# nadult/Snail

Measured on AMD Instinct MI355X. Metric: Mrays/sec (primary), higher is better.
Workload: dtype f32; 1 GPU; BASELINE config 1: atrium (263124 tris, sponza.obj stand-in) 1920x1080 primary rays, hit records (t,u,v,triId); reflections=False, arith=host_sse, arith_tables=host CPU, packets=16x16 px = 1 wavefront, bvh_nodes=161677, bvh_depth=21, frames_in_flight=16, frames_per_launch=4, launches_in_flight=4, settle_frames=348, order_refresh=16, ranks=1, packet_order=heaviest first (node visits of an earlier frame), parallelism=single-gpu

## Files before the change

include/snail_hip_debug.h:

```cpp
#ifndef SNAIL_HIP_DEBUG_H
#define SNAIL_HIP_DEBUG_H
#include "snail_hip.h"
#ifdef __cplusplus
extern "C" {
#endif

int snail_debug_delay_dev(float microseconds, void *stream);

int snail_debug_clock_dev(float microseconds, uint64_t *d_out2, void *stream);

int snail_debug_recip_check(uint64_t out2[2]);

int snail_debug_hostsse_device_check(int fn, int threads, uint64_t *badChunks, uint32_t *firstBadChunk);

int snail_debug_dispatch_rate(int blocks, int threads, int reps, float *ms_per_launch);

int snail_debug_anyorder(SnailScene *, const float cam[13], int resx, int resy, int frames, int flags, float *ms_total);

int snail_debug_occupancy(int out[4]);

int snail_debug_rel_flag_count(SnailScene *, const float org[3], int *count);

#ifdef __cplusplus
}
#endif
#endif
```

snail_amd/_lib.py:

```python
from __future__ import annotations

import ctypes as C
import os

HERE = os.path.dirname(os.path.abspath(__file__))
LIB_PATH = os.environ.get("SNAIL_LIB_PATH") or os.path.join(HERE, "libsnailhip.so")


class SnailError(RuntimeError):
    pass


_lib = None

_VP, _I, _F13 = C.c_void_p, C.c_int, C.c_void_p
SIGNATURES = {
    "snail_last_error": (C.c_char_p, []),
    "snail_device_count": (_I, []),
    "snail_tris_from_verts": (_I, [_VP, _I, _VP]),
    "snail_bvh_build": (_I, [_VP, _I, _VP, _VP, _VP, _VP]),
    "snail_scene_create": (_VP, [_VP, _I, _VP, _I, _I, _I]),
    "snail_scene_destroy": (None, [_VP]),
    "snail_scene_info": (_I, [_VP, _VP, _VP, _VP, _VP]),
    "snail_scene_flags": (_I, [_VP, _VP, _VP]),
    "snail_scene_set_arith": (_I, [_VP, _I]),
    "snail_scene_arith": (_I, [_VP, _VP]),
    "snail_host_sse_tables": (_I, [_VP]),
    "snail_arith_set_tables": (_I, [_VP]),
    "snail_arith_prepare_device": (_I, []),
    "snail_host_sse_check": (_I, [_I, C.c_uint64, C.c_uint64, _I, _VP, _VP]),
    "snail_scene_create_lbvh": (_VP, [_VP, _I, _I, _I, _VP, _VP]),
    "snail_scene_download": (_I, [_VP, _VP, _VP]),
    "snail_trace_primary": (_I, [_VP, _F13, _I, _I, _I, _I, _I, _I, _VP, _VP, _VP, _VP, _VP]),
    "snail_trace_frame_packets": (_I, [_VP, _F13, _I, _I, _VP, _VP, _VP, _VP, _VP]),
    "snail_trace_primary_dev": (_I, [_VP, _F13, _I, _I, _I, _I, _I, _I, _VP, _VP, _VP, _VP, _VP, _VP]),
    "snail_trace_packets_dev": (_I, [_VP, _F13, _I, _I, _VP, _I, _VP, _VP, _VP, _VP, _VP, _VP]),
    "snail_trace_packets_shaded_dev": (_I, [_VP, _F13, _I, _I, _VP, _I, _VP, _VP, _VP]),
    "snail_trace_primary_batch_dev": (_I, [_VP, _I, _VP, _I, _I, _VP, _VP, _VP, _VP, _VP, _VP, _VP, _VP]),
    "snail_trace_packets_shaded_batch_dev": (_I, [_VP, _I, _VP, _I, _I, _VP, _I, _VP, _VP, _VP]),
    "snail_trace_primary_batch_reorder_dev": (_I, [_VP, _I, _VP, _I, _I, _VP, _VP, _VP, _VP, _VP, _VP, _VP, _VP, _I, _VP]),
    "snail_render_whitted_reorder_dev": (_I, [_VP, _F13, _I, _I, _VP, _I, _VP, _VP, _I, _VP, _I, _VP, _VP, _VP, _VP, _I, _VP]),
    "snail_primary_slots": (_I, [_I, _I]),
    "snail_trace_primary_ordered_dev": (_I, [_VP, _F13, _I, _I, _I, _I, _I, _I, _VP, _VP, _VP, _VP, _VP, _VP, _VP, _VP]),
    "snail_trace_packets_ordered_dev": (_I, [_VP, _F13, _I, _I, _VP, _I, _VP, _VP, _VP, _VP, _VP, _VP, _VP, _VP]),
    "snail_order_from_cost_dev": (_I, [_VP, _I, _VP, _VP]),
    "snail_order_from_cost_hint_dev": (_I, [_VP, _I, _VP, _I, _VP]),
    "snail_packets_to_frame_dev": (_I, [_VP, _I, _I, _I, _VP, _VP, _VP, _VP, _VP, _VP, _VP, _VP, _VP]),
    "snail_trace_rays": (_I, [_VP, _I, _I, _I, _VP, _VP, _VP, _VP, _VP, _VP, _VP, _VP]),
    "snail_trace_rays_dev": (_I, [_VP, _I, _I, _I, _VP, _VP, _VP, _VP, _VP, _VP, _VP, _VP, _VP]),
    "snail_trace_shadow": (_I, [_VP, _I, _I, _VP, _VP, _VP, _VP, _VP]),
    "snail_trace_shadow_dev": (_I, [_VP, _I, _I, _VP, _VP, _VP, _VP, _VP, _VP]),
    "snail_shade_depth_dev": (_I, [_VP, _I, _VP, _VP]),
    "snail_shade_depth_arith_dev": (_I, [_VP, _I, _VP, _I, _VP]),
    "snail_packets_bgr_to_frame_dev": (_I, [_VP, _I, _I, _I, _VP, _VP, _I, _VP]),
    "snail_packets_bgr_to_frame_chunked_dev": (_I, [_VP, _I, _I, C.c_int64, _I, _I, _VP, _VP, _I, _VP]),
    "snail_packets_bgr_to_planar_dev": (_I, [_VP, _VP, _VP, _I, _VP, _VP, _VP]),
    "snail_planar_to_frame_dev": (_I, [_VP, _VP, _I, _VP, _VP, _I, _I, _I, _VP]),
    "snail_render_whitted_dev": (_I, [_VP, _F13, _I, _I, _VP, _I, _VP, _VP, _I, _VP, _I, _VP, _VP]),
    "snail_render_whitted_ordered_dev": (_I, [_VP, _F13, _I, _I, _VP, _I, _VP, _VP, _I, _VP, _I, _VP, _VP, _VP, _VP]),
    "snail_render_whitted_packets_dev": (_I, [_VP, _F13, _I, _I, _VP, _I, _VP, _I, _VP, _VP, _I, _VP, _VP, _VP]),
    "snail_trace_transparency_dev": (_I, [_VP, _F13, _I, _I, _VP, _I, _VP, _VP, _VP, _VP, _I, _VP, _VP, _VP, _VP, _VP]),
    "snail_render_tiles": (_I, [_VP, _F13, _I, _I, _VP, _VP, _I, _VP, _I, _VP, _VP, _I, _VP, _VP]),
    "snail_render_tiles_multi": (_I, [_VP, _I, _F13, _I, _I, _VP, _VP, _I, _VP, _I, _VP, _VP, _I, _VP, _VP]),
    "snail_render_image": (_I, [_VP, _F13, _I, _I, _VP, _I, _VP, _VP, _I, _VP, _I, _VP]),
    "snail_account_primary": (_I, [_VP, _F13, _I, _I, _I, _I, _I, _I, _VP]),
    "snail_account_packets": (_I, [_VP, _F13, _I, _I, _VP]),
    "snail_last_launch": (_I, [_VP, _VP, _VP]),
}

INSTANCES_SIGNATURES = {
    "snail_instances_build": (_I, [_VP, _VP, _I, _VP, _I, _VP, _VP, _VP, _VP]),
    "snail_instances_create": (_VP, [_VP, _I, _VP, _I, _VP, _VP, _I, _I]),
    "snail_instances_update": (_I, [_VP, _VP, _I, _VP, _VP, _I, _I, _VP]),
    "snail_instances_destroy": (None, [_VP]),
    "snail_instances_trace_primary_dev": (_I, [_VP, _F13, _I, _I, _I, _I, _I, _I, _VP, _VP, _VP, _VP, _VP, _VP, _VP]),
    "snail_instances_trace_packets_dev": (_I, [_VP, _F13, _I, _I, _VP, _I, _VP, _VP, _VP, _VP, _VP, _VP, _VP]),
    "snail_instances_trace_rays_dev": (_I, [_VP, _I, _I, _I, _VP, _VP, _VP, _VP, _VP, _VP, _VP, _VP, _VP, _VP]),
    "snail_instances_trace_shadow_dev": (_I, [_VP, _I, _I, _VP, _VP, _VP, _VP, _VP, _VP]),
    "snail_instances_trace_rays": (_I, [_VP, _I, _I, _I, _VP, _VP, _VP, _VP, _VP, _VP, _VP, _VP, _VP]),
    "snail_instances_trace_shadow": (_I, [_VP, _I, _I, _VP, _VP, _VP, _VP, _VP]),
    "snail_instances_trace_frame_packets": (_I, [_VP, _F13, _I, _I, _VP, _VP, _VP, _VP, _VP, _VP]),
    "snail_instances_render_depth": (_I, [_VP, _F13, _I, _I, _VP, _I, _VP]),
}

INSTANCES_SHADE_SIGNATURES = {
    "snail_instances_render_whitted_dev": (_I, [_VP, _F13, _I, _I, _VP, _I, _VP, _VP, _I, _VP, _I, _VP, _VP]),
    "snail_instances_render_whitted_packets_dev": (_I, [_VP, _F13, _I, _I, _VP, _I, _VP, _I, _VP, _VP, _I, _VP, _VP, _VP]),
    "snail_instances_render_image": (_I, [_VP, _F13, _I, _I, _VP, _I, _VP, _VP, _I, _VP, _I, _VP]),
}

INSTANCES_TILES_SIGNATURES = {
    "snail_instances_shade_packets_dev": (_I, [_VP, _F13, _I, _I, _VP, _I, _VP, _I, _VP, _VP, _I, _VP, _VP, _VP, _VP]),
    "snail_instances_render_tiles": (_I, [_VP, _F13, _I, _I, _VP, _VP, _I, _VP, _I, _VP, _VP, _I, _VP, _VP, _VP]),
    "snail_instances_render_frame": (_I, [_VP, _F13, _I, _I, _VP, _I, _VP, _VP, _I, _VP, _I, _VP]),
}

INSTANCES_BUILD_SIGNATURES = {
    "snail_instances_rebuild_dev": (_I, [_VP, _VP, _VP, _I, _VP, _VP, _VP]),
    "snail_instances_read_tree": (_I, [_VP, _VP, _I, _VP, _VP, _VP, _I, _VP]),
}

BVH_FAST_SIGNATURES = {
    "snail_bvh_build_fast": (_I, [_VP, _I, _VP, _VP, _VP, _VP]),
    "snail_scene_create_fast_dev": (_VP, [_VP, _I, _I, _VP, _VP, _VP]),
    "snail_scene_rebuild_fast_dev": (_I, [_VP, _VP, _I, _VP, _VP, _VP]),
}

HEATMAP_SIGNATURES = {
    "snail_packet_stats_dev": (_I, [_VP, _F13, _I, _I, _VP, _I, _VP, _I, _I, _VP, _VP, _VP]),
    "snail_render_heat_packets_dev": (_I, [_VP, _F13, _I, _I, _VP, _I, _VP, _I, _I, _VP, _VP, _VP, _VP]),
    "snail_render_heat_tiles": (_I, [_VP, _F13, _I, _I, _VP, _VP, _I, _VP, _I, _I, _VP, _VP]),
    "snail_render_heat_image": (_I, [_VP, _F13, _I, _I, _VP, _I, _I, _VP, _I, _VP]),
    "snail_instances_packet_stats_dev": (_I, [_VP, _F13, _I, _I, _VP, _I, _VP, _I, _I, _VP, _VP, _VP]),
    "snail_instances_heat_packets_dev": (_I, [_VP, _F13, _I, _I, _VP, _I, _VP, _I, _I, _VP, _VP, _VP, _VP, _VP]),
    "snail_instances_render_heat_tiles": (_I, [_VP, _F13, _I, _I, _VP, _VP, _I, _VP, _I, _I, _VP, _VP, _VP]),
    "snail_instances_render_heat_frame": (_I, [_VP, _F13, _I, _I, _VP, _I, _I, _VP, _I, _VP]),
}

MATERIALS_SIGNATURES = {
    "snail_shtris_pack": (_I, [_VP, _VP, _VP, _VP, _I, _VP, _VP]),
    "snail_texture_size": (C.c_int64, [_I, _I, _VP]),
    "snail_texture_build": (_I, [_VP, _I, _I, _VP, C.c_int64, _VP]),
    "snail_materials_create": (_VP, [_VP, _VP, _I, _VP, _I, _VP, _I, _VP, _I]),
    "snail_materials_destroy": (None, [_VP]),
    "snail_materials_shade_packets_dev": (_I, [_VP, _F13, _I, _I, _VP, _I, _VP, _VP, _VP, _VP, _VP, _VP]),
    "snail_render_materials_dev": (_I, [_VP, _F13, _I, _I, _VP, _I, _VP, _I, _VP, _I, _VP, _VP]),
    "snail_render_materials_packets_dev": (_I, [_VP, _F13, _I, _I, _VP, _I, _VP, _I, _VP, _I, _VP, _VP, _VP]),
    "snail_render_materials_image": (_I, [_VP, _F13, _I, _I, _VP, _I, _VP, _I, _VP, _I, _VP]),
}

MATERIALS_BOUNCE_SIGNATURES = {
    "snail_materials_mirror_packets_dev": (_I, [_VP, _F13, _I, _I, _VP, _I, _VP, _VP, _VP, _VP, _VP, _VP, _VP, _VP, _VP, _VP]),
    "snail_materials_shade_rays_dev": (_I, [_VP, _I, _VP, _VP, _VP, _VP, _VP, _VP, _VP, _VP]),
    "snail_materials_bounce_dev": (_I, [_VP, _F13, _I, _I, _VP, _I, _VP, _I, _VP, _I, _VP, _VP]),
    "snail_materials_bounce_packets_dev": (_I, [_VP, _F13, _I, _I, _VP, _I, _VP, _I, _VP, _I, _VP, _VP, _VP]),
    "snail_materials_bounce_image": (_I, [_VP, _F13, _I, _I, _VP, _I, _VP, _I, _VP, _I, _VP]),
}

MATERIALS_TILES_SIGNATURES = {
    "snail_materials_frame_packets_dev": (_I, [_VP, _F13, _I, _I, _VP, _I, _VP, _I, _VP, _I, _VP, _VP, _VP, _VP]),
    "snail_materials_render_tiles": (_I, [_VP, _F13, _I, _I, _VP, _VP, _I, _VP, _I, _VP, _I, _VP, _VP, _VP]),
    "snail_materials_render_frame": (_I, [_VP, _F13, _I, _I, _VP, _I, _VP, _I, _VP, _I, _VP]),
}

DEBUG_SIGNATURES = {
    "snail_debug_delay_dev": (_I, [C.c_float, _VP]),
    "snail_debug_clock_dev": (_I, [C.c_float, _VP, _VP]),
    "snail_debug_recip_check": (_I, [_VP]),
    "snail_debug_dispatch_rate": (_I, [_I, _I, _I, _VP]),
    "snail_debug_hostsse_device_check": (_I, [_I, _I, _VP, _VP]),
    "snail_debug_occupancy": (_I, [_VP]),
    "snail_debug_anyorder": (_I, [_VP, _F13, _I, _I, _I, _I, _VP]),
    "snail_debug_rel_flag_count": (_I, [_VP, _VP, _VP]),
}
DEBUG_LIB_PATH = os.path.join(HERE, "libsnailhip_debug.so")
_dbg = None


def debug_lib():
    global _dbg
    if _dbg is None:
        if not os.path.exists(DEBUG_LIB_PATH):
            raise SnailError("workbench library %s is missing: `make -C snail_amd/csrc debug`" % DEBUG_LIB_PATH)
        L = C.CDLL(DEBUG_LIB_PATH)
        for table in (SIGNATURES, INSTANCES_SIGNATURES, INSTANCES_SHADE_SIGNATURES, INSTANCES_TILES_SIGNATURES, INSTANCES_BUILD_SIGNATURES, BVH_FAST_SIGNATURES, HEATMAP_SIGNATURES, MATERIALS_SIGNATURES, MATERIALS_BOUNCE_SIGNATURES, MATERIALS_TILES_SIGNATURES, DEBUG_SIGNATURES):
            for name, (res, args) in table.items():
                fn = getattr(L, name)
                fn.restype = res
                fn.argtypes = args
        _dbg = L
    return _dbg


def lib():
    global _lib
    if _lib is None:
        if not os.path.exists(LIB_PATH):
            raise SnailError(
                "HIP extension %s is missing: run `python -c 'import __graft_entry__ as g; g.build()'` "
                "(or `make -C snail_amd/csrc`). There is no CPU fallback." % LIB_PATH)
        try:
            L = C.CDLL(LIB_PATH)
        except OSError as e:
            raise SnailError("cannot load %s: %s" % (LIB_PATH, e)) from e
        for table in (SIGNATURES, INSTANCES_SIGNATURES, INSTANCES_SHADE_SIGNATURES, INSTANCES_TILES_SIGNATURES, INSTANCES_BUILD_SIGNATURES, BVH_FAST_SIGNATURES, HEATMAP_SIGNATURES, MATERIALS_SIGNATURES, MATERIALS_BOUNCE_SIGNATURES, MATERIALS_TILES_SIGNATURES):
            for name, (res, args) in table.items():
                fn = getattr(L, name)
                fn.restype = res
                fn.argtypes = args
        for name, (res, args) in DEBUG_SIGNATURES.items():
            fn = getattr(L, name, None)
            if fn is not None:
                fn.restype = res
                fn.argtypes = args
        _lib = L
    return _lib


def check(rc: int, what: str) -> None:
    if rc != 0:
        msg = lib().snail_last_error()
        raise SnailError("%s failed (status %d): %s" % (what, rc, msg.decode() if msg else "?"))


def ptr(a):
    if a is None:
        return None
    if hasattr(a, "data_ptr"):
        return C.c_void_p(a.data_ptr())
    return a.ctypes.data_as(C.c_void_p)
```

snail_amd/csrc/bvh_fast.inc:

```
namespace devf {

using devb::BuildHdr;
using devb::TNode;
static_assert(SNAIL_MAX_DEPTH == devb::kMaxDepth, "BuildHdr::qCount and the small kernel's stack are sized for DBVH::maxDepth == BVH::maxDepth");

struct FastArgs : devb::SplitArgs {
	const float *verts;
	uint4 *nodes, *pf, *tris;
	unsigned trisOff;
	int needSane;
	int *cur;
	int *perm, *info;
};

__global__ void k_fast_init(FastArgs A) {
	const int i = blockIdx.x * blockDim.x + threadIdx.x;
	if(i < A.n) A.startCnt[i] = 0;
	if(i == 0) devb::hdrInit(*A.hdr);
}

__global__ void k_fast_boxes(FastArgs A) {
	const int i = blockIdx.x * blockDim.x + threadIdx.x;
	if(i >= A.n) return;
	float p[9], rec[16];
// ... 13 lines not shown
	for(int k = 0; k < 3; k++) { o[k] = lo[k]; o[3 + k] = hi[k]; }
	A.src[i] = i;
	for(int k = 0; k < 3; k++) { devb::keyMin(&A.hdr->rootMin[k], lo[k], i); devb::keyMax(&A.hdr->rootMax[k], hi[k], i); }
}

__global__ void k_fast_commit(FastArgs A) {
	const BuildHdr &H = *A.hdr;
	const int g = blockIdx.x * blockDim.x + threadIdx.x, stride = gridDim.x * blockDim.x;
	const int status = H.status != 0 ? H.status : (A.needSane && H.insane) ? 3 : 0;
	if(status != 0) {
		if(g == 0 && A.info) { A.info[0] = status; A.info[1] = 0; A.info[2] = 0; A.info[3] = A.n; }
		return;
	}
	const int nTemp = H.nTemp;
	for(int t = g; t < nTemp; t += stride) {
		const TNode nd = A.tn[t];
		const int idx = t == 0 ? 0 : 1 + 2 * (A.startCnt[nd.pfirst] + nd.pchain) + nd.side;
		const unsigned sub = nd.inner ? (unsigned)(1 + 2 * (A.startCnt[nd.first] + nd.chain)) : ((unsigned)nd.first | 0x80000000u);
		const unsigned in[8] = {__float_as_uint(nd.lo[0]), __float_as_uint(nd.lo[1]), __float_as_uint(nd.lo[2]), __float_as_uint(nd.hi[0]),
								__float_as_uint(nd.hi[1]), __float_as_uint(nd.hi[2]), sub, (unsigned)nd.aux};
		A.nodes[(size_t)idx * 2] = make_uint4(in[0], in[1], in[2], in[3]);
		A.nodes[(size_t)idx * 2 + 1] = make_uint4(in[4], in[5], in[6], in[7]);
		if(A.pf) {
			unsigned out[8];
			dev::pfEncode(in, out, A.trisOff);
			A.pf[(size_t)(idx + 1) * 2] = make_uint4(out[0], out[1], out[2], out[3]);
			A.pf[(size_t)(idx + 1) * 2 + 1] = make_uint4(out[4], out[5], out[6], out[7]);
		}
	}
	for(int i = g; i < A.n; i += stride) {
		const int s = A.src[i];
		float p[9], rec[16];
		for(int k = 0; k < 9; k++) p[k] = A.verts[(size_t)s * 9 + k];
		(void)dev::lbvh::triRecord(p, rec);
		uint4 *o = A.tris + (size_t)i * 4;
		for(int q = 0; q < 4; q++)
			o[q] = make_uint4(__float_as_uint(rec[q * 4]), __float_as_uint(rec[q * 4 + 1]), __float_as_uint(rec[q * 4 + 2]), __float_as_uint(rec[q * 4 + 3]));
		if(A.perm) A.perm[i] = s;
	}
	if(g == 0) {
		const int nNodes = 1 + 2 * H.totalInner;
		A.cur[0] = nNodes; A.cur[1] = H.depth; A.cur[2] = H.insane ? 0 : 1; A.cur[3] = 0;
		if(A.info) { A.info[0] = 0; A.info[1] = nNodes; A.info[2] = H.depth; A.info[3] = A.n; }
	}
}

}

struct SnailSceneFast {
	char *base = nullptr;
	int *dCur = nullptr;
	int cur[4] = {0, 0, 0, 0};
	bool curOnDevice = false;
	int depthLimit = SNAIL_MAX_DEPTH;
	hipEvent_t ready = nullptr;
	bool hasReady = false;
	struct Use { hipStream_t stream; hipEvent_t ev; };
	std::vector<Use> uses;
};

namespace {

void fastFree(SnailSceneFast *f) {
	if(!f) return;
	if(f->base) (void)hipFree(f->base);
	if(f->dCur) (void)hipFree(f->dCur);
	if(f->ready) (void)hipEventDestroy(f->ready);
	for(auto &u : f->uses) (void)hipEventDestroy(u.ev);
	delete f;
}

int fastSceneBegin(SnailScene *s, hipStream_t stream) {
	SnailSceneFast *f = s->fast;
	if(f->hasReady) HIP_TRY(hipStreamWaitEvent(stream, f->ready, 0));
	return 0;
}
void fastSceneEnd(SnailScene *s, hipStream_t stream) {
	SnailSceneFast *f = s->fast;
	for(auto &u : f->uses)
		if(u.stream == stream) { (void)hipEventRecord(u.ev, stream); return; }
	SnailSceneFast::Use u;
	u.stream = stream;
	if(hipEventCreateWithFlags(&u.ev, hipEventDisableTiming) != hipSuccess) return;
	(void)hipEventRecord(u.ev, stream);
	f->uses.push_back(u);
}

int fastEnqueue(SnailScene *s, const float *dVerts, int32_t *dPerm, int32_t *dInfo, int needSane, hipStream_t st) {
	SnailSceneFast *f = s->fast;
	const int n = s->nTris;
	devf::FastArgs A;
	memset((void *)&A, 0, sizeof(A));
	buildCarve(f->base, n, A);
	A.n = n; A.maxDepth = f->depthLimit;
	A.verts = dVerts;
	A.nodes = s->dNodes; A.tris = s->dTris; A.pf = s->pfOKButNesting ? (uint4 *)s->dPF : nullptr; A.trisOff = (unsigned)s->trisOff;
	A.needSane = needSane; A.cur = f->dCur; A.perm = dPerm; A.info = dInfo;
	const devb::SplitArgs &SA = A;
	typedef devb::SplitBvh P;
	const int perN = (n + 255) / 256;
	hipLaunchKernelGGL(devf::k_fast_init, dim3(perN), dim3(256), 0, st, A);
	hipLaunchKernelGGL(devf::k_fast_boxes, dim3(perN), dim3(256), 0, st, A);
	hipLaunchKernelGGL(devb::k_build_root<P>, dim3(1), dim3(64), 0, st, SA);
	if(n > devb::kSmall) {
		const int most = n / (devb::kSmall + 1) + 1;
		const int wide = 28;
		for(int level = 0; level < wide; level++) {
			const int grid = std::min(level < 11 ? (1 << level) : 2048, most);
			hipLaunchKernelGGL(devb::k_build_big<P>, dim3(grid), dim3(256), 0, st, SA, level, level + 1);
		}
		hipLaunchKernelGGL(devb::k_build_big<P>, dim3(1), dim3(256), 0, st, SA, wide, (int)devb::kLevels);
	}
	if(n >= P::minSplit) hipLaunchKernelGGL(devb::k_build_small<P>, dim3(std::min(n / 2 + 1, 8192)), dim3(64), 0, st, SA);
	hipLaunchKernelGGL(devb::k_build_scan, dim3(1), dim3(1024), 0, st, SA);
	hipLaunchKernelGGL(devf::k_fast_commit, dim3((unsigned)std::min((2 * (long long)n + 255) / 256, 4096LL)), dim3(256), 0, st, A);
	HIP_TRY(hipGetLastError());
	if(!f->ready) HIP_TRY(hipEventCreateWithFlags(&f->ready, hipEventDisableTiming));
	HIP_TRY(hipEventRecord(f->ready, st));
	f->hasReady = true;
	f->curOnDevice = true;
	return 0;
}

int fastCurrent(const SnailScene *cs, int cur[4]) {
	SnailScene *s = const_cast<SnailScene *>(cs);
	SnailSceneFast *f = s->fast;
	DeviceGuard guard(s->device);
	std::lock_guard<std::mutex> lock(s->mu);
	if(f->curOnDevice) {
		if(f->hasReady) HIP_TRY(hipEventSynchronize(f->ready));
		HIP_TRY(hipMemcpy(f->cur, f->dCur, sizeof(f->cur), hipMemcpyDeviceToHost));
		f->curOnDevice = false;
	}
	memcpy(cur, f->cur, sizeof(f->cur));
	return 0;
}

}

extern "C" {

SnailScene *snail_scene_create_fast_dev(const float *d_verts9, int nTris, int device, int32_t *d_perm, int32_t *d_info, void *stream) {
	const char *fn = "snail_scene_create_fast_dev";
	if(!d_verts9 || nTris <= 0 || nTris > (1 << 29)) { snail_set_error("%s: bad arguments", fn); return nullptr; }
	DeviceGuard guard(device);
	if(!guard.ok) { snail_set_error("%s: hipSetDevice(%d) failed", fn, device); return nullptr; }
	hipStream_t st = (hipStream_t)stream;
	SnailScene *s = new SnailScene();
	s->fast = new SnailSceneFast();
	SnailSceneFast *f = s->fast;
	const int cap = 2 * nTris - 1;
	s->device = device; s->nNodes = cap; s->nTris = nTris;
	const size_t trisOff = pfTrisOffset(cap), pfBytes = trisOff + (size_t)nTris * 64;
	const bool fits = (size_t)cap + 1 < ((size_t)1 << 20) && pfBytes < ((size_t)1 << 31);
	s->trisOff = (int)(fits ? trisOff : 0);
	s->pfOKButNesting = fits ? 1 : 0;
	hipError_t e;
	if((e = hipMalloc((void **)&s->dNodes, (size_t)cap * 32)) != hipSuccess || (e = hipMalloc((void **)&s->dPF, fits ? pfBytes : (size_t)nTris * 64)) != hipSuccess ||
	   (e = hipMalloc((void **)&f->base, buildScratchBytes(nTris))) != hipSuccess || (e = hipMalloc((void **)&f->dCur, 4 * sizeof(int))) != hipSuccess ||
	   (fits && (e = hipMemset(s->dPF, 0, ((size_t)cap + 1) * 32)) != hipSuccess) || (e = hipMemset(f->dCur, 0, 4 * sizeof(int))) != hipSuccess) {
		snail_set_error("%s: %s", fn, hipGetErrorString(e));
		snail_scene_destroy(s);
		return nullptr;
	}
	s->dTris = (uint4 *)(s->dPF + s->trisOff);
	hipLaunchKernelGGL(dev::lbvh::k_fill_empty, dim3((unsigned)((cap + 255) / 256)), dim3(256), 0, 0, (float *)s->dNodes, cap);
	int cur[4] = {0, 0, 0, 0}, status[8] = {0};
	if((e = hipDeviceSynchronize()) != hipSuccess || fastEnqueue(s, d_verts9, d_perm, d_info, 0, st) != 0 || (e = hipStreamSynchronize(st)) != hipSuccess ||
	   (e = hipMemcpy(status, f->base, sizeof(status), hipMemcpyDeviceToHost)) != hipSuccess || fastCurrent(s, cur) != 0) {
		if(e != hipSuccess) snail_set_error("%s: %s", fn, hipGetErrorString(e));
		snail_scene_destroy(s);
		return nullptr;
	}
	if(status[0] != 0) {
		if(status[0] == 1) snail_set_error("%s: a vertex is not finite", fn);
		else snail_set_error("%s: the tree is deeper than BVH::maxDepth = %d", fn, SNAIL_MAX_DEPTH);
		snail_scene_destroy(s);
		return nullptr;
	}
	s->depth = cur[1]; s->fastOK = cur[2]; s->nestedOK = 1; s->pfOK = s->pfOKButNesting;
	f->depthLimit = s->depth > 62 ? SNAIL_MAX_DEPTH : 62;
	return s;
}

int snail_scene_rebuild_fast_dev(SnailScene *s, const float *d_verts9, int nTris, int32_t *d_perm, int32_t *d_info, void *stream) {
	const char *fn = "snail_scene_rebuild_fast_dev";
	if(int rc = checkScene(s, fn)) return rc;
	if(!s->fast) { snail_set_error("%s: the handle was not made by snail_scene_create_fast_dev", fn); return 1; }
	if(!d_verts9 || nTris != s->nTris) { snail_set_error("%s: %d triangles, the handle holds %d (or null vertices)", fn, nTris, s->nTris); return 1; }
	hipStream_t st = (hipStream_t)stream;
	DeviceGuard guard(s->device);
	SNAIL_LOCK(s);
	SnailSceneFast *f = s->fast;
	for(auto &u : f->uses) HIP_TRY(hipStreamWaitEvent(st, u.ev, 0));
	if(f->hasReady) HIP_TRY(hipStreamWaitEvent(st, f->ready, 0));
	for(auto &e : s->rel) e.valid = false;
	return fastEnqueue(s, d_verts9, d_perm, d_info, s->fastOK, st);
}

}
```

snail_amd/csrc/snail_dev.inc:

```
namespace SNAIL_DEV_NS {

typedef unsigned long long u64;
typedef unsigned u32x4 __attribute__((ext_vector_type(4)));
typedef const __attribute__((address_space(4))) u32x4 *scalar_ptr;

struct Node {
	float bmin[3], bmax[3];
	unsigned sub;
	int aux;
};

__device__ __forceinline__ float asf(unsigned u) { return __uint_as_float(u); }
__device__ __forceinline__ float asf(int u) { return __int_as_float(u); }

typedef const __attribute__((address_space(4))) char *scalar_bytes;
__device__ __forceinline__ Node loadNode(const uint4 *nodes, int idx) {
	const unsigned off = (unsigned)idx << 5;
	scalar_ptr p = (scalar_ptr)((scalar_bytes)(unsigned long long)nodes + off);
	u32x4 a = p[0], b = p[1];
	Node n;
	n.bmin[0] = asf(a.x); n.bmin[1] = asf(a.y); n.bmin[2] = asf(a.z);
	n.bmax[0] = asf(a.w); n.bmax[1] = asf(b.x); n.bmax[2] = asf(b.y);
	n.sub = b.z; n.aux = (int)b.w;
	return n;
// ... 721 lines not shown
		const int farIdx = (int)n.sub + (firstNode ^ 1);
		const Node nn = loadNode(nodes, nearIdx);

		auto fastPass = [&](const Node &n) -> u64 {
			float tn[4], tf[4];
			if(M == M_COH) {
				float pn[3], pf[3];
#pragma unroll
				for(int k = 0; k < 3; k++) {
					const int lo = __float_as_int(n.bmin[k]), hi = __float_as_int(n.bmax[k]);
					const int sw = (lo ^ hi) & octMask[k];
					pn[k] = __int_as_float(lo ^ sw); pf[k] = __int_as_float(hi ^ sw);
					if(SHARED) { pn[k] = pn[k] - org[k][0]; pf[k] = pf[k] - org[k][0]; }
				}
#pragma unroll
				for(int l = 0; l < 4; l++) {
					float lo[3], hi[3];
#pragma unroll
					for(int k = 0; k < 3; k++) {
						lo[k] = Q.id[k][l] * (SHARED ? pn[k] : pn[k] - org[k][l]);
						hi[k] = Q.id[k][l] * (SHARED ? pf[k] : pf[k] - org[k][l]);
					}
					tn[l] = vmax3(lo[0], lo[1], lo[2]);
					tf[l] = vmin3(hi[0], hi[1], hi[2]);
				}
			} else {
				float pn[3], pf[3];
#pragma unroll
				for(int k = 0; k < 3; k++) { pn[k] = SHARED ? n.bmin[k] - org[k][0] : n.bmin[k]; pf[k] = SHARED ? n.bmax[k] - org[k][0] : n.bmax[k]; }
#pragma unroll
				for(int l = 0; l < 4; l++) {
					float lo[3], hi[3];
#pragma unroll
					for(int k = 0; k < 3; k++) {
						const float a = Q.id[k][l] * (SHARED ? pn[k] : pn[k] - org[k][l]);
						const float b = Q.id[k][l] * (SHARED ? pf[k] : pf[k] - org[k][l]);
						lo[k] = vmin(a, b); hi[k] = vmax(a, b);
					}
					tn[l] = vmax3(lo[0], lo[1], lo[2]);
					tf[l] = vmin3(hi[0], hi[1], hi[2]);
				}
			}
			if(DISTPOS) {
#pragma unroll
				for(int l = 0; l < 4; l++) { tn[l] = vmax(tn[l], 0.0f); tf[l] = vmin(tf[l], Q.dist[l]); }
				const float slack = vmax3(tf[0] - tn[0], tf[1] - tn[1], vmax(tf[2] - tn[2], tf[3] - tn[3]));
				return __builtin_amdgcn_ballot_w64(slack >= 0.0f);
			} else {
				float sl[4];
#pragma unroll
				for(int l = 0; l < 4; l++) sl[l] = vmin(vmin(tf[l], Q.dist[l]) - tn[l], tf[l]);
				const float slack = vmax3(sl[0], sl[1], vmax(sl[2], sl[3]));
				return __builtin_amdgcn_ballot_w64(slack >= 0.0f);
			}
				};
		u64 passMask = 0;
		if(EXACT) {
			bool anyPass = false;
			if(boxTestInterval(n, iv)) {
				float tmn[3], tmx[3];
				if(SHARED) {
#pragma unroll
					for(int k = 0; k < 3; k++) { tmn[k] = n.bmin[k] - org[k][0]; tmx[k] = n.bmax[k] - org[k][0]; }
				}
#pragma unroll
				for(int l = 0; l < 4; l++) {
					float lmin = 0.0f, lmax = 0.0f;
#pragma unroll
					for(int k = 0; k < 3; k++) {
						float l1 = Q.id[k][l] * (SHARED ? tmn[k] : n.bmin[k] - org[k][l]);
						float l2 = Q.id[k][l] * (SHARED ? tmx[k] : n.bmax[k] - org[k][l]);
						float lo = Min<M_EXACT>(l1, l2), hi = Max<M_EXACT>(l1, l2);
						if(k == 0) { lmin = lo; lmax = hi; }
						else if(SHADOW) { lmin = Max<M_EXACT>(lo, lmin); lmax = Min<M_EXACT>(hi, lmax); }
						else { lmin = Max<M_EXACT>(lmin, lo); lmax = Min<M_EXACT>(lmax, hi); }
					}
					bool pass = SHADOW ? (lmax >= 0.0f && lmin <= Min<M_EXACT>(lmax, Q.dist[l])) : !(lmax < 0.0f || lmin > Min<M_EXACT>(lmax, Q.dist[l]));
					anyPass |= pass;
				}
			}
			passMask = __builtin_amdgcn_ballot_w64(anyPass);
		} else passMask = fastPass(n);
		const u64 alive = passMask & __builtin_amdgcn_ballot_w64((unsigned)(lane - first) <= (unsigned)(last - first));
		if(alive != 0) {
			first = __builtin_ctzll(alive);
			last = 63 - __builtin_clzll(alive);
			if(!isLeaf) {
				const int fl = first | (last << 8);
				if(!DEEP || sp < 64) writeLane2(stkNode, farIdx, stkFL, fl, sp);
				else writeLane2(stkNode2, farIdx, stkFL2, fl, sp - 64);
				sp++;
				n = nn;
				continue;
			}
		const int count = n.aux, firstTri = (int)(n.sub & 0x7fffffffu);
		if(SHARED) {
			if(leafShared<MASK, SHADOW, M, BARY>(tris, count, firstTri, size, lane, first, last, org, Q, mask4, tid, bu, bv, iv, st)) return;
		} else {
			leafPerRay<MASK, M, BARY>(tris, count, firstTri, lane, first, last, org, Q, mask4, tid, bu, bv, st);
		}
		}
		if(sp == 0) break;
		sp--;
		int cur, fl;
		if(!DEEP || sp < 64) { cur = __builtin_amdgcn_readlane(stkNode, sp); fl = __builtin_amdgcn_readlane(stkFL, sp); }
		else { cur = __builtin_amdgcn_readlane(stkNode2, sp - 64); fl = __builtin_amdgcn_readlane(stkFL2, sp - 64); }
		first = fl & 0xff; last = fl >> 8;
		n = loadNode(nodes, cur);
	}
}

#define SNAIL_SLAB_COH(L, NX, FX, NY, FY, NZ, FZ)                                                                                           \
	"v_mul_f32 %[t0], %[ix" L "], %[pnx]\n v_mul_f32 %[t1], %[iy" L "], %[pny]\n v_mul_f32 %[t2], %[iz" L "], %[pnz]\n"                    \
	"v_mul_f32 %[t3], %[ix" L "], %[pfx]\n v_mul_f32 %[t4], %[iy" L "], %[pfy]\n v_mul_f32 %[t5], %[iz" L "], %[pfz]\n"                    \
	"v_max3_f32 %[t0], %[t0], %[t1], %[t2]\n v_min3_f32 %[t3], %[t3], %[t4], %[t5]\n"
#define SNAIL_SLAB_FAST(L, NX, FX, NY, FY, NZ, FZ)                                                                                          \
	"v_mul_f32 %[t0], %[ix" L "], %[pnx]\n v_mul_f32 %[t3], %[ix" L "], %[pfx]\n v_min_f32 %[u0], %[t0], %[t3]\n v_max_f32 %[t3], %[t0], %[t3]\n" \
	"v_mul_f32 %[t1], %[iy" L "], %[pny]\n v_mul_f32 %[t4], %[iy" L "], %[pfy]\n v_min_f32 %[t0], %[t1], %[t4]\n v_max_f32 %[t4], %[t1], %[t4]\n" \
	"v_mul_f32 %[t2], %[iz" L "], %[pnz]\n v_mul_f32 %[t5], %[iz" L "], %[pfz]\n v_min_f32 %[t1], %[t2], %[t5]\n v_max_f32 %[t5], %[t2], %[t5]\n" \
	"v_max3_f32 %[t0], %[u0], %[t0], %[t1]\n v_min3_f32 %[t3], %[t3], %[t4], %[t5]\n"
#define SNAIL_SLAB_COH_R(L, NX, FX, NY, FY, NZ, FZ)                                                                                         \
	"v_mul_f32 %[t0], " NX ", %[ix" L "]\n v_mul_f32 %[t1], " NY ", %[iy" L "]\n v_mul_f32 %[t2], " NZ ", %[iz" L "]\n"                    \
	"v_mul_f32 %[t3], " FX ", %[ix" L "]\n v_mul_f32 %[t4], " FY ", %[iy" L "]\n v_mul_f32 %[t5], " FZ ", %[iz" L "]\n"                    \
	"v_max3_f32 %[t0], %[t0], %[t1], %[t2]\n v_min3_f32 %[t3], %[t3], %[t4], %[t5]\n"
#define SNAIL_SLAB_FAST_R(L, NX, FX, NY, FY, NZ, FZ)                                                                                        \
	"v_mul_f32 %[t0], " NX ", %[ix" L "]\n v_mul_f32 %[t3], " FX ", %[ix" L "]\n v_min_f32 %[u0], %[t0], %[t3]\n v_max_f32 %[t3], %[t0], %[t3]\n" \
	"v_mul_f32 %[t1], " NY ", %[iy" L "]\n v_mul_f32 %[t4], " FY ", %[iy" L "]\n v_min_f32 %[t0], %[t1], %[t4]\n v_max_f32 %[t4], %[t1], %[t4]\n" \
	"v_mul_f32 %[t2], " NZ ", %[iz" L "]\n v_mul_f32 %[t5], " FZ ", %[iz" L "]\n v_min_f32 %[t1], %[t2], %[t5]\n v_max_f32 %[t5], %[t2], %[t5]\n" \
	"v_max3_f32 %[t0], %[u0], %[t0], %[t1]\n v_min3_f32 %[t3], %[t3], %[t4], %[t5]\n"
#define SNAIL_SLABO_COH(L, NX, FX, NY, FY, NZ, FZ)                                                                                          \
	"v_sub_f32 %[t0], " NX ", %[ox" L "]\n v_sub_f32 %[t1], " NY ", %[oy" L "]\n v_sub_f32 %[t2], " NZ ", %[oz" L "]\n"                    \
	"v_sub_f32 %[t3], " FX ", %[ox" L "]\n v_sub_f32 %[t4], " FY ", %[oy" L "]\n v_sub_f32 %[t5], " FZ ", %[oz" L "]\n"                    \
	"v_mul_f32 %[t0], %[ix" L "], %[t0]\n v_mul_f32 %[t1], %[iy" L "], %[t1]\n v_mul_f32 %[t2], %[iz" L "], %[t2]\n"                       \
	"v_mul_f32 %[t3], %[ix" L "], %[t3]\n v_mul_f32 %[t4], %[iy" L "], %[t4]\n v_mul_f32 %[t5], %[iz" L "], %[t5]\n"                       \
	"v_max3_f32 %[t0], %[t0], %[t1], %[t2]\n v_min3_f32 %[t3], %[t3], %[t4], %[t5]\n"
#define SNAIL_SLABO_FAST(L, NX, FX, NY, FY, NZ, FZ)                                                                                         \
	"v_sub_f32 %[t0], " NX ", %[ox" L "]\n v_sub_f32 %[t3], " FX ", %[ox" L "]\n v_mul_f32 %[t0], %[ix" L "], %[t0]\n v_mul_f32 %[t3], %[ix" L "], %[t3]\n" \
	"v_min_f32 %[u0], %[t0], %[t3]\n v_max_f32 %[t3], %[t0], %[t3]\n"                                                                      \
	"v_sub_f32 %[t1], " NY ", %[oy" L "]\n v_sub_f32 %[t4], " FY ", %[oy" L "]\n v_mul_f32 %[t1], %[iy" L "], %[t1]\n v_mul_f32 %[t4], %[iy" L "], %[t4]\n" \
	"v_min_f32 %[t0], %[t1], %[t4]\n v_max_f32 %[t4], %[t1], %[t4]\n"                                                                      \
	"v_sub_f32 %[t2], " NZ ", %[oz" L "]\n v_sub_f32 %[t5], " FZ ", %[oz" L "]\n v_mul_f32 %[t2], %[iz" L "], %[t2]\n v_mul_f32 %[t5], %[iz" L "], %[t5]\n" \
	"v_min_f32 %[t1], %[t2], %[t5]\n v_max_f32 %[t5], %[t2], %[t5]\n"                                                                      \
	"v_max3_f32 %[t0], %[u0], %[t0], %[t1]\n v_min3_f32 %[t3], %[t3], %[t4], %[t5]\n"
#define SNAIL_PRE_SHARED(NX, FX, NY, FY, NZ, FZ)                                                                                            \
	" v_sub_f32 %[pnx], " NX ", %[ox]\n v_sub_f32 %[pny], " NY ", %[oy]\n v_sub_f32 %[pnz], " NZ ", %[oz]\n"                               \
	" v_sub_f32 %[pfx], " FX ", %[ox]\n v_sub_f32 %[pfy], " FY ", %[oy]\n v_sub_f32 %[pfz], " FZ ", %[oz]\n"
#define SNAIL_PRE_NONE(NX, FX, NY, FY, NZ, FZ) ""
#define SNAIL_ORG_SHARED() [ox] "v"(org[0][0]), [oy] "v"(org[1][0]), [oz] "v"(org[2][0])
#define SNAIL_ORG_PERRAY()                                                                                                                 \
	[ox0] "v"(org[0][0]), [ox1] "v"(org[0][1]), [ox2] "v"(org[0][2]), [ox3] "v"(org[0][3]), [oy0] "v"(org[1][0]), [oy1] "v"(org[1][1]),     \
		[oy2] "v"(org[1][2]), [oy3] "v"(org[1][3]), [oz0] "v"(org[2][0]), [oz1] "v"(org[2][1]), [oz2] "v"(org[2][2]), [oz3] "v"(org[2][3])
#define SNAIL_TAIL_POS(L, S) "v_max_f32 %[t0], 0, %[t0]\n v_min_f32 %[t3], %[t3], %[d" L "]\n v_sub_f32 %[" S "], %[t3], %[t0]\n"
#define SNAIL_TAIL_ANY(L, S) "v_min_f32 %[t4], %[t3], %[d" L "]\n v_sub_f32 %[t4], %[t4], %[t0]\n v_min_f32 %[" S "], %[t4], %[t3]\n"
#define SNAIL_POP_2W                                                                                                                       \
	" v_readlane_b32 %[cur], %[stkN], %[sp]\n v_readlane_b32 %[fl], %[stkF], %[sp]\n"                                                      \
	" s_and_b32 %[first], %[fl], 0xff\n s_lshr_b32 %[last], %[fl], 8\n"
#define SNAIL_PUSH_2W                                                                                                                      \
	" s_lshl_b32 %[off], %[last], 8\n s_or_b32 %[off], %[off], %[first]\n"                                                                 \
	" s_mov_b32 m0, %[sp]\n v_writelane_b32 %[stkN], %[fl], m0\n v_writelane_b32 %[stkF], %[off], m0\n"
#define SNAIL_COUNT " s_add_u32 %[cnt], %[cnt], 1\n"
#define SNAIL_DRAIN_SMEM " s_waitcnt lgkmcnt(0)\n"
#define SNAIL_DESCEND_ASM(PRE, ORGOPS, SLAB, TAIL, CNTPOP, CNTVISIT, NX, FX, NY, FY, NZ, FZ)                                                 \
	asm volatile(SNAIL_DRAIN_SMEM                                                                                                          \
				 "L_pop_%=:\n"                                                                                                             \
				 " s_cmp_eq_u32 %[sp], 0\n s_cbranch_scc1 L_done_%=\n"                                                                     \
				 " s_sub_u32 %[sp], %[sp], 1\n" CNTPOP                                                                                     \
				 SNAIL_POP_2W                                                                                                              \
				 " s_lshl_b32 %[off], %[cur], 5\n s_load_dwordx8 s[84:91], %[base], %[off]\n"                                              \
				 " s_sub_u32 %[width], %[last], %[first]\n"                                                                                \
				 " s_bfm_b64 exec, %[width], %[first]\n s_bitset1_b64 exec, %[last]\n"                                                     \
				 " s_waitcnt lgkmcnt(0)\n"                                                                                                 \
				 "L_visit_%=:\n" CNTVISIT                                                                                                  \
				 PRE(NX, FX, NY, FY, NZ, FZ)                                                                                               \
				 SLAB("0", NX, FX, NY, FY, NZ, FZ) TAIL("0", "s0") SLAB("1", NX, FX, NY, FY, NZ, FZ) TAIL("1", "s1")                       \
				 SLAB("2", NX, FX, NY, FY, NZ, FZ) TAIL("2", "s2") SLAB("3", NX, FX, NY, FY, NZ, FZ) TAIL("3", "s3")                       \
				 " v_max_f32 %[s2], %[s2], %[s3]\n v_max3_f32 %[s0], %[s0], %[s1], %[s2]\n"                                                \
				 " v_cmp_le_f32 vcc, 0, %[s0]\n"                                                                                           \
				 " s_and_b64 %[alive], vcc, exec\n s_cbranch_scc0 L_pop_%=\n"                                                              \
				 " s_ff1_i32_b64 %[first], %[alive]\n s_flbit_i32_b64 %[last], %[alive]\n s_xor_b32 %[last], %[last], 63\n"                \
				 " s_sub_u32 %[width], %[last], %[first]\n"                                                                                \
				 " s_bfm_b64 exec, %[width], %[first]\n s_bitset1_b64 exec, %[last]\n"                                                     \
				 " s_cmp_lt_i32 s90, 0\n s_cbranch_scc1 L_leaf_%=\n"                                                                       \
				 " s_lshr_b32 %[cur], %[sign16], s91\n s_xor_b32 %[cur], %[cur], s91\n s_bfe_u32 %[cur], %[cur], 0x10010\n"                \
				 " s_add_u32 %[fl], s90, 1\n s_sub_u32 %[fl], %[fl], %[cur]\n"                                                             \
				 " s_add_u32 %[cur], s90, %[cur]\n s_lshl_b32 %[off], %[cur], 5\n"                                                         \
				 " s_load_dwordx8 s[84:91], %[base], %[off]\n"                                                                             \
				 SNAIL_PUSH_2W                                                                                                             \
				 " s_add_u32 %[sp], %[sp], 1\n"                                                                                            \
				 " s_waitcnt lgkmcnt(0)\n s_branch L_visit_%=\n"                                                                           \
				 "L_leaf_%=:\n s_mov_b32 %[leafSub], s90\n s_mov_b32 %[leafAux], s91\n s_branch L_end_%=\n"                                \
				 "L_done_%=:\n s_mov_b32 %[leafSub], 0\n s_mov_b32 %[leafAux], 0\n"                                                        \
				 "L_end_%=:\n s_mov_b64 exec, -1\n"                                                                                        \
				 : [sp] "+s"(sp), [first] "+s"(first), [last] "+s"(last), [cnt] "+s"(cnt), [stkN] "+v"(stkN), [stkF] "+v"(stkF),           \
				   [leafSub] "=&s"(leafSub), [leafAux] "=&s"(leafAux), [cur] "=&s"(sCur), [fl] "=&s"(sFl), [off] "=&s"(sOff),              \
				   [width] "=&s"(sWidth), [rng] "=&s"(sRng), [alive] "=&s"(sAlive), [pnx] "=&v"(vt[0]), [pny] "=&v"(vt[1]),                \
				   [pnz] "=&v"(vt[2]), [pfx] "=&v"(vt[3]), [pfy] "=&v"(vt[4]), [pfz] "=&v"(vt[5]), [t0] "=&v"(vt[6]), [t1] "=&v"(vt[7]),   \
				   [t2] "=&v"(vt[8]), [t3] "=&v"(vt[9]), [t4] "=&v"(vt[10]), [t5] "=&v"(vt[11]), [s0] "=&v"(vt[12]), [s1] "=&v"(vt[13]),   \
				   [s2] "=&v"(vt[14]), [s3] "=&v"(vt[15]), [u0] "=&v"(vt[16])                                                              \
				 : [base] "s"(nodeBase), [sign16] "s"(sign16), [lane] "v"(lane), ORGOPS(), [ix0] "v"(Q.id[0][0]), [ix1] "v"(Q.id[0][1]), [ix2] "v"(Q.id[0][2]), [ix3] "v"(Q.id[0][3]),        \
				   [iy0] "v"(Q.id[1][0]), [iy1] "v"(Q.id[1][1]), [iy2] "v"(Q.id[1][2]), [iy3] "v"(Q.id[1][3]), [iz0] "v"(Q.id[2][0]),      \
				   [iz1] "v"(Q.id[2][1]), [iz2] "v"(Q.id[2][2]), [iz3] "v"(Q.id[2][3]), [d0] "v"(Q.dist[0]), [d1] "v"(Q.dist[1]),          \
				   [d2] "v"(Q.dist[2]), [d3] "v"(Q.dist[3])                                                                                \
				 : "s84", "s85", "s86", "s87", "s88", "s89", "s90", "s91", "vcc", "scc", "m0");                                            \
	              \
	asm volatile("" ::"s"(sp), "s"(first), "s"(last), "s"(cnt), "v"(stkN), "v"(stkF), "s"(leafSub), "s"(leafAux), "s"(sCur), "s"(sFl), "s"(sOff),    \
				 "s"(sWidth), "s"(sRng), "s"(sAlive), "v"(vt[0]), "v"(vt[1]), "v"(vt[2]), "v"(vt[3]), "v"(vt[4]), "v"(vt[5]), "v"(vt[6]), "v"(vt[7]), \
				 "v"(vt[8]), "v"(vt[9]), "v"(vt[10]), "v"(vt[11]), "v"(vt[12]), "v"(vt[13]), "v"(vt[14]), "v"(vt[15]), "v"(vt[16]))
#define SNAIL_REL_INSIDE_BIT 31
#define SNAIL_MOV_REC(D0, D1, D2, D3, S0, S1, S2, S3)                                                                                       \
	" s_mov_b64 " D0 ", " S0 "\n s_mov_b64 " D1 ", " S1 "\n s_mov_b64 " D2 ", " S2 "\n s_mov_b64 " D3 ", " S3 "\n"
#define SNAIL_A_FROM_T SNAIL_MOV_REC("s[84:85]", "s[86:87]", "s[88:89]", "s[90:91]", "s[68:69]", "s[70:71]", "s[72:73]", "s[74:75]")
#define SNAIL_PF_LEAFREQ_TRI(OTHERSET) " s_bitset0_b32 %[cur], 31\n s_load_dwordx8 " OTHERSET ", %[base], %[cur]\n"
#define SNAIL_PF_LEAFREQ_SLOT0(OTHERSET) " s_max_i32 %[cur], %[cur], 0\n s_load_dwordx8 " OTHERSET ", %[base], %[cur]\n"

#define SNAIL_PF2_NEARFAR(SUB, AUX, FARX, OTHERSET, LEAFREQ)                                                                                          \
				 " s_and_b32 %[cur], " AUX ", %[sign16]\n s_cselect_b32 %[cur], 32, 0\n"                                                       \
				 " s_xor_b32 %[cur], " SUB ", %[cur]\n s_xor_b32 " FARX ", %[cur], 32\n"                                                       \
				 LEAFREQ(OTHERSET)
#define SNAIL_PF2_TAIL(X, SUB)  \
				 " v_max_f32 %[s2], %[s2], %[s3]\n v_max3_f32 %[s0], %[s0], %[s1], %[s2]\n"                                                \
				 " v_cmpx_le_f32 vcc, 0, %[s0]\n"                                                                                           \
				 " s_cbranch_execz L_fail_%=\n"                                                                                            \
				 " s_cbranch_scc1 L_leaf" X "_%=\n"
#define SNAIL_PF2_ISLEAF(SUB) " s_cmp_lt_i32 " SUB ", 0\n"
#define SNAIL_PF2_ALIVE " s_sub_u32 %[cur], %[last], %[first]\n s_bfm_b64 %[alive], %[cur], %[first]\n s_bitset1_b64 %[alive], %[last]\n"
#define SNAIL_PF2_FIRSTLAST " s_ff1_i32_b64 %[first], exec\n s_flbit_i32_b64 %[last], exec\n s_xor_b32 %[last], %[last], 63\n"
static_assert(SNAIL_REL_INSIDE_BIT == 31, "SNAIL_OIN_TEST_SNAIL_TAIL_POS names the bit in its text");
#define SNAIL_OIN_TEST_SNAIL_TAIL_POS(AUX, LBL) " s_bitcmp1_b32 " AUX ", 31\n s_cbranch_scc1 " LBL "_%=\n"
#define SNAIL_OIN_TEST_SNAIL_TAIL_ANY(AUX, LBL) ""
#define SNAIL_OIN_TEST_of(TAIL) SNAIL_OIN_TEST_##TAIL
#define SNAIL_OIN_PENDING(X, Y, OTHERSET, SUB, AUX, FARX, FARY, CNTVISIT, LEAFREQ)                                                          \
				 "L_oin" X "p_%=:\n" CNTVISIT                                          \
				 SNAIL_PF2_NEARFAR(SUB, AUX, FARX, OTHERSET, LEAFREQ)                                                                        \
				 SNAIL_PF2_FIRSTLAST                                                           \
				 " s_lshl_b32 %[off], %[last], 6\n s_or_b32 %[off], %[off], %[first]\n s_lshl_b32 %[off], %[off], 20\n"                    \
				 SNAIL_PF2_ALIVE                                                                                                            \
				 " s_lshr_b32 %[topw], " FARY ", 5\n s_or_b32 %[topw], %[topw], %[off]\n"                                                    \
				 " v_writelane_b32 %[stkN], %[topw], m0\n s_add_u32 m0, m0, 1\n"                                                            \
				 " s_branch L_visit" Y "p_%=\n"
#define SNAIL_OIN_COPIES_SNAIL_TAIL_POS(CNTVISIT, LEAFREQ)                                                                                  \
				 "L_oinAq_%=:\n" CNTVISIT                                                 \
				 " s_and_b32 %[cur], %[topw], 0xfffff\n s_lshl_b32 %[off], %[cur], 5\n"                                                    \
				 " s_load_dwordx8 s[68:75], %[base], %[off]\n"                                                                             \
				 SNAIL_PF2_NEARFAR("s90", "s91", "%[fl]", "s[76:83]", LEAFREQ)                                                               \
				 " s_bfe_u32 %[first], %[topw], 0x60014\n s_lshr_b32 %[last], %[topw], 26\n" SNAIL_PF2_ALIVE                               \
				 " s_branch L_visitBp_%=\n"                                                                                                \
				 SNAIL_OIN_PENDING("B", "A", "s[84:91]", "s82", "s83", "%[width]", "%[fl]", CNTVISIT, LEAFREQ)                               \
				 SNAIL_OIN_PENDING("A", "B", "s[76:83]", "s90", "s91", "%[fl]", "%[width]", CNTVISIT, LEAFREQ)
#define SNAIL_OIN_COPIES_SNAIL_TAIL_ANY(CNTVISIT, LEAFREQ) ""
#define SNAIL_OIN_COPIES_of(TAIL) SNAIL_OIN_COPIES_##TAIL
#define SNAIL_PF2_PENDING(X, OTHERSET, SUB, AUX, FARX, FARY, PRE, SLAB, TAIL, CNTVISIT, LEAFREQ, NX, FX, NY, FY, NZ, FZ)                                                   \
				 "L_visit" X "p_%=:\n"                                                                                                      \
				 " s_waitcnt lgkmcnt(0)\n"                                                 \
				 " s_load_dwordx8 s[68:75], %[base], " FARY "\n"                              \
				 SNAIL_OIN_TEST_of(TAIL)(AUX, "L_oin" X "p")                                                                                  \
				 CNTVISIT PRE(NX, FX, NY, FY, NZ, FZ)                                                                                        \
				 SLAB("0", NX, FX, NY, FY, NZ, FZ) TAIL("0", "s0")                                                                           \
				 SNAIL_PF2_NEARFAR(SUB, AUX, FARX, OTHERSET, LEAFREQ)                                                                        \
				 SLAB("1", NX, FX, NY, FY, NZ, FZ) TAIL("1", "s1")                                                                           \
				 SNAIL_PF2_FIRSTLAST                                                      \
				 " s_lshl_b32 %[off], %[last], 6\n s_or_b32 %[off], %[off], %[first]\n s_lshl_b32 %[off], %[off], 20\n"                    \
				 SNAIL_PF2_ALIVE                                                                                                            \
				 SLAB("2", NX, FX, NY, FY, NZ, FZ) TAIL("2", "s2")                                                                           \
				 " s_lshr_b32 %[topw], " FARY ", 5\n s_or_b32 %[topw], %[topw], %[off]\n"                                                    \
				 " v_writelane_b32 %[stkN], %[topw], m0\n s_add_u32 m0, m0, 1\n" SNAIL_PF2_ISLEAF(SUB)                                       \
				 SLAB("3", NX, FX, NY, FY, NZ, FZ) TAIL("3", "s3")                                                                           \
				 SNAIL_PF2_TAIL(X, SUB)
#define SNAIL_PF2_LEAF(X, SUB, AUX)                                                                                                         \
				 "L_leaf" X "_%=:\n" SNAIL_PF2_FIRSTLAST                                                                                    \
				 " s_bfe_u32 %[leafSub], " SUB ", 0x190006\n s_sub_u32 %[leafSub], %[leafSub], 0x80000\n s_bitset1_b32 %[leafSub], 31\n"   \
				 " s_mov_b32 %[leafAux], " AUX "\n s_waitcnt lgkmcnt(0)\n s_branch L_end_%=\n"
#define SNAIL_DESCEND_PF2X(EXTRACLOB, PREVARS, PRE, ORGOPS, SLAB, TAIL, CNTPOP, CNTVISIT, LEAFREQ, NXA, FXA, NYA, FYA, NZA, FZA, NXB, FXB, NYB, FYB, NZB, FZB)                                                  \
	asm volatile(SNAIL_DRAIN_SMEM " s_mov_b32 m0, %[sp]\n"                                                                                \
				 "L_entry_%=:\n"                                                                                                           \
				 " s_cmp_eq_u32 m0, 0\n s_cbranch_scc1 L_done_%=\n"                                                                     \
				 " s_sub_u32 %[off], m0, 1\n"                                                                                           \
				 " v_readlane_b32 %[topw], %[stkN], %[off]\n"                                                                              \
				 " s_and_b32 %[cur], %[topw], 0xfffff\n s_lshl_b32 %[off], %[cur], 5\n"                                                    \
				 " s_load_dwordx8 s[68:75], %[base], %[off]\n"                                                                             \
				 " s_bfe_u32 %[first], %[topw], 0x60014\n s_lshr_b32 %[last], %[topw], 26\n" SNAIL_PF2_ALIVE                               \
				 "L_pop_%=:\n"                             \
				 " s_sub_u32 m0, m0, 1\n" CNTPOP                                                                                     \
				 " s_mov_b64 exec, %[alive]\n"                                                                                             \
				 " s_waitcnt lgkmcnt(0)\n" SNAIL_A_FROM_T                                                                                  \
				                   \
				 " s_sub_u32 %[off], m0, 1\n s_max_i32 %[off], %[off], 0\n"   \
				 " v_readlane_b32 %[topw], %[stkN], %[off]\n"                                                                              \
				 SNAIL_OIN_TEST_of(TAIL)("s91", "L_oinAq")                                                                                  \
				 CNTVISIT PRE(NXA, FXA, NYA, FYA, NZA, FZA)                                                                                 \
				 SLAB("0", NXA, FXA, NYA, FYA, NZA, FZA) TAIL("0", "s0")                                                          \
				 " s_and_b32 %[cur], %[topw], 0xfffff\n s_lshl_b32 %[off], %[cur], 5\n"                                                    \
				 " s_load_dwordx8 s[68:75], %[base], %[off]\n"                                                                             \
				 SLAB("1", NXA, FXA, NYA, FYA, NZA, FZA) TAIL("1", "s1")                                                          \
				 SNAIL_PF2_NEARFAR("s90", "s91", "%[fl]", "s[76:83]", LEAFREQ)                                                                       \
				 SLAB("2", NXA, FXA, NYA, FYA, NZA, FZA) TAIL("2", "s2")                                                          \
				 " s_bfe_u32 %[first], %[topw], 0x60014\n s_lshr_b32 %[last], %[topw], 26\n" SNAIL_PF2_ALIVE SNAIL_PF2_ISLEAF("s90")        \
				 SLAB("3", NXA, FXA, NYA, FYA, NZA, FZA) TAIL("3", "s3")                                                          \
				 SNAIL_PF2_TAIL("A", "s90")                                                                                                 \
				                                                                    \
				 SNAIL_PF2_PENDING("B", "s[84:91]", "s82", "s83", "%[width]", "%[fl]", PRE, SLAB, TAIL, CNTVISIT, LEAFREQ, NXB, FXB, NYB, FYB, NZB, FZB)                   \
				                                                                    \
				 SNAIL_PF2_PENDING("A", "s[76:83]", "s90", "s91", "%[fl]", "%[width]", PRE, SLAB, TAIL, CNTVISIT, LEAFREQ, NXA, FXA, NYA, FYA, NZA, FZA)                   \
				 " s_branch L_visitBp_%=\n"                                                                                                \
				 SNAIL_PF2_LEAF("A", "s90", "s91") SNAIL_PF2_LEAF("B", "s82", "s83")                                                       \
				 SNAIL_OIN_COPIES_of(TAIL)(CNTVISIT, LEAFREQ)                                                                               \
				 "L_fail_%=:\n"                                                                                                            \
				 " s_cmp_eq_u32 m0, 0\n s_cbranch_scc0 L_pop_%=\n"                                                                      \
				 "L_done_%=:\n s_mov_b32 %[leafSub], 0\n s_mov_b32 %[leafAux], 0\n s_waitcnt lgkmcnt(0)\n"                                  \
				 "L_end_%=:\n s_mov_b64 exec, -1\n s_mov_b32 %[sp], m0\n"                                                                                        \
				 : [sp] "+s"(sp), [first] "+s"(first), [last] "+s"(last), [cnt] "+s"(cnt), [stkN] "+v"(stkN), [stkF] "+v"(stkF),           \
				   [leafSub] "=&s"(leafSub), [leafAux] "=&s"(leafAux), [cur] "=&s"(sCur), [fl] "=&s"(sFl), [off] "=&s"(sOff),              \
				   [width] "=&s"(sWidth), [topw] "=&s"(sTopw), [alive] "=&s"(sAlive), PREVARS() [t0] "=&v"(vt[6]), [t1] "=&v"(vt[7]),   \
				   [t2] "=&v"(vt[8]), [t3] "=&v"(vt[9]), [t4] "=&v"(vt[10]), [t5] "=&v"(vt[11]), [s0] "=&v"(vt[12]), [s1] "=&v"(vt[13]),   \
				   [s2] "=&v"(vt[14]), [s3] "=&v"(vt[15]), [u0] "=&v"(vt[16])                                                              \
				 : [base] "s"(nodeBase), [sign16] "s"(sign16), [lane] "v"(lane), ORGOPS(), [ix0] "v"(Q.id[0][0]), [ix1] "v"(Q.id[0][1]), [ix2] "v"(Q.id[0][2]), [ix3] "v"(Q.id[0][3]),        \
				   [iy0] "v"(Q.id[1][0]), [iy1] "v"(Q.id[1][1]), [iy2] "v"(Q.id[1][2]), [iy3] "v"(Q.id[1][3]), [iz0] "v"(Q.id[2][0]),      \
				   [iz1] "v"(Q.id[2][1]), [iz2] "v"(Q.id[2][2]), [iz3] "v"(Q.id[2][3]), [d0] "v"(Q.dist[0]), [d1] "v"(Q.dist[1]),          \
				   [d2] "v"(Q.dist[2]), [d3] "v"(Q.dist[3])                                                                                \
				 : "s68", "s69", "s70", "s71", "s72", "s73", "s74", "s75", "s76", "s77", "s78", "s79", "s80", "s81", "s82", "s83", "s84", "s85", "s86", "s87", \
				   "s88", "s89", "s90", "s91", "vcc", "scc", "m0" EXTRACLOB);                                                                        \
	asm volatile("" ::"s"(sp), "s"(first), "s"(last), "s"(cnt), "v"(stkN), "v"(stkF), "s"(leafSub), "s"(leafAux), "s"(sCur), "s"(sFl), "s"(sOff),    \
				 "s"(sWidth), "s"(sTopw), "s"(sAlive), "v"(vt[6]), "v"(vt[7]), \
				 "v"(vt[8]), "v"(vt[9]), "v"(vt[10]), "v"(vt[11]), "v"(vt[12]), "v"(vt[13]), "v"(vt[14]), "v"(vt[15]), "v"(vt[16]))
#define SNAIL_PREVARS_SHARED() [pnx] "=&v"(vt[0]), [pny] "=&v"(vt[1]), [pnz] "=&v"(vt[2]), [pfx] "=&v"(vt[3]), [pfy] "=&v"(vt[4]), [pfz] "=&v"(vt[5]),
#define SNAIL_PREVARS_NONE() [pnx] "=&v"(vt[0]), [pny] "=&v"(vt[1]), [pnz] "=&v"(vt[2]), [pfx] "=&v"(vt[3]), [pfy] "=&v"(vt[4]), [pfz] "=&v"(vt[5]),
#define SNAIL_PREVARS_SNAIL_PRE_SHARED SNAIL_PREVARS_SHARED
#define SNAIL_PREVARS_SNAIL_PRE_NONE SNAIL_PREVARS_NONE
#define SNAIL_PREVARS_SNAIL_PRE_SEL SNAIL_PREVARS_NONE
#define SNAIL_PREVARS_EMPTY()
#define SNAIL_PRE_NONE_X(NX, FX, NY, FY, NZ, FZ) ""
#define SNAIL_PREVARS_SNAIL_PRE_NONE_X SNAIL_PREVARS_EMPTY
#define SNAIL_PREVARS_of(PRE) SNAIL_PREVARS_##PRE
#define SNAIL_DESCEND_PF2(PRE, ORGOPS, SLAB, TAIL, CNTPOP, CNTVISIT, LEAFREQ, NXA, FXA, NYA, FYA, NZA, FZA, NXB, FXB, NYB, FYB, NZB, FZB)                 \
	SNAIL_DESCEND_PF2X(, SNAIL_PREVARS_of(PRE), PRE, ORGOPS, SLAB, TAIL, CNTPOP, CNTVISIT, LEAFREQ, NXA, FXA, NYA, FYA, NZA, FZA, NXB, FXB, NYB, FYB, NZB, FZB)
#define SNAIL_PRE_SEL(NX, FX, NY, FY, NZ, FZ)                                                                                               \
				 " s_bitcmp1_b32 %[sign16], 8\n s_cselect_b32 s62, " FX ", " NX "\n s_cselect_b32 s65, " NX ", " FX "\n"                       \
				 " s_bitcmp1_b32 %[sign16], 9\n s_cselect_b32 s63, " FY ", " NY "\n s_cselect_b32 s66, " NY ", " FY "\n"                       \
				 " s_bitcmp1_b32 %[sign16], 10\n s_cselect_b32 s64, " FZ ", " NZ "\n s_cselect_b32 s67, " NZ ", " FZ "\n"
#define SNAIL_SLABO_SEL(L, NX, FX, NY, FY, NZ, FZ) SNAIL_SLABO_COH(L, "s62", "s65", "s63", "s66", "s64", "s67")
#define SNAIL_SEL_CLOB , "s62", "s63", "s64", "s65", "s66", "s67"
#define SNAIL_DESCEND_PF2_SEL(ORGOPS, SLAB, TAIL, CNTPOP, CNTVISIT, LEAFREQ)                                                                \
	SNAIL_DESCEND_PF2X(SNAIL_SEL_CLOB, SNAIL_PREVARS_NONE, SNAIL_PRE_SEL, ORGOPS, SLAB, TAIL, CNTPOP, CNTVISIT, LEAFREQ, "s84", "s87", "s85", "s88", "s86", "s89", "s76", "s79", "s77", "s80", "s78", "s81")
#define SNAIL_DESCEND_PF2_PLAIN(PRE, ORGOPS, SLAB, TAIL, CNTPOP, CNTVISIT, LEAFREQ) SNAIL_DESCEND_PF2(PRE, ORGOPS, SLAB, TAIL, CNTPOP, CNTVISIT, LEAFREQ, "s84", "s87", "s85", "s88", "s86", "s89", "s76", "s79", "s77", "s80", "s78", "s81")
#define SNAIL_DESCEND_PF2_OCT(PRE, ORGOPS, SLAB, TAIL, CNTPOP, CNTVISIT, LEAFREQ, OCT)                                                                                                    \
	switch(OCT) {                                                                                                                          \
	case 0: SNAIL_DESCEND_PF2(PRE, ORGOPS, SLAB, TAIL, CNTPOP, CNTVISIT, LEAFREQ, "s84", "s87", "s85", "s88", "s86", "s89", "s76", "s79", "s77", "s80", "s78", "s81"); break;            \
	case 1: SNAIL_DESCEND_PF2(PRE, ORGOPS, SLAB, TAIL, CNTPOP, CNTVISIT, LEAFREQ, "s87", "s84", "s85", "s88", "s86", "s89", "s79", "s76", "s77", "s80", "s78", "s81"); break;            \
	case 2: SNAIL_DESCEND_PF2(PRE, ORGOPS, SLAB, TAIL, CNTPOP, CNTVISIT, LEAFREQ, "s84", "s87", "s88", "s85", "s86", "s89", "s76", "s79", "s80", "s77", "s78", "s81"); break;            \
	case 3: SNAIL_DESCEND_PF2(PRE, ORGOPS, SLAB, TAIL, CNTPOP, CNTVISIT, LEAFREQ, "s87", "s84", "s88", "s85", "s86", "s89", "s79", "s76", "s80", "s77", "s78", "s81"); break;            \
	case 4: SNAIL_DESCEND_PF2(PRE, ORGOPS, SLAB, TAIL, CNTPOP, CNTVISIT, LEAFREQ, "s84", "s87", "s85", "s88", "s89", "s86", "s76", "s79", "s77", "s80", "s81", "s78"); break;            \
	case 5: SNAIL_DESCEND_PF2(PRE, ORGOPS, SLAB, TAIL, CNTPOP, CNTVISIT, LEAFREQ, "s87", "s84", "s85", "s88", "s89", "s86", "s79", "s76", "s77", "s80", "s81", "s78"); break;            \
	case 6: SNAIL_DESCEND_PF2(PRE, ORGOPS, SLAB, TAIL, CNTPOP, CNTVISIT, LEAFREQ, "s84", "s87", "s88", "s85", "s89", "s86", "s76", "s79", "s80", "s77", "s81", "s78"); break;            \
	default: SNAIL_DESCEND_PF2(PRE, ORGOPS, SLAB, TAIL, CNTPOP, CNTVISIT, LEAFREQ, "s87", "s84", "s88", "s85", "s89", "s86", "s79", "s76", "s80", "s77", "s81", "s78"); break;           \
	}

#define SNAIL_DESCEND_OCT(PRE, ORGOPS, SLAB, TAIL, CNTPOP, CNTVISIT, OCT)                                                                     \
	switch(OCT) {                                                                                                                          \
	case 0: SNAIL_DESCEND_ASM(PRE, ORGOPS, SLAB, TAIL, CNTPOP, CNTVISIT, "s84", "s87", "s85", "s88", "s86", "s89"); break;                              \
	case 1: SNAIL_DESCEND_ASM(PRE, ORGOPS, SLAB, TAIL, CNTPOP, CNTVISIT, "s87", "s84", "s85", "s88", "s86", "s89"); break;                              \
	case 2: SNAIL_DESCEND_ASM(PRE, ORGOPS, SLAB, TAIL, CNTPOP, CNTVISIT, "s84", "s87", "s88", "s85", "s86", "s89"); break;                              \
	case 3: SNAIL_DESCEND_ASM(PRE, ORGOPS, SLAB, TAIL, CNTPOP, CNTVISIT, "s87", "s84", "s88", "s85", "s86", "s89"); break;                              \
	case 4: SNAIL_DESCEND_ASM(PRE, ORGOPS, SLAB, TAIL, CNTPOP, CNTVISIT, "s84", "s87", "s85", "s88", "s89", "s86"); break;                              \
	case 5: SNAIL_DESCEND_ASM(PRE, ORGOPS, SLAB, TAIL, CNTPOP, CNTVISIT, "s87", "s84", "s85", "s88", "s89", "s86"); break;                              \
	case 6: SNAIL_DESCEND_ASM(PRE, ORGOPS, SLAB, TAIL, CNTPOP, CNTVISIT, "s84", "s87", "s88", "s85", "s89", "s86"); break;                              \
	default: SNAIL_DESCEND_ASM(PRE, ORGOPS, SLAB, TAIL, CNTPOP, CNTVISIT, "s87", "s84", "s88", "s85", "s89", "s86"); break;                             \
	}

template <bool SHADOW, bool COH, bool PACK, bool MASK, bool BARY, bool POSDIST, bool REL = true >
__device__ __forceinline__ void walkSharedAsm(const uint4 *__restrict__ nodes , const uint4 *__restrict__ tris, int size, int lane,
											  const float (&org)[3][4], Quad &Q, unsigned mask4, int (&tid)[4], float (&bu)[4], float (&bv)[4], float *lds,
											  Counters &st, const int oct) {
	Interval iv;
	{
		unsigned act4 = lane < size ? 15u : 0u;
		if(SHADOW) {
			act4 = 0;
			if(lane < size)
#pragma unroll
				for(int l = 0; l < 4; l++) act4 |= (Q.dist[l] >= 0.0f ? 1u : 0u) << l;
		} else if(MASK) act4 = lane < size ? (mask4 & 15u) : 0u;
		computeMinMax<false, (MASK || SHADOW)>(Q.d, act4, size, lane, lds, iv.minDir, iv.maxDir);
	}
#pragma unroll
	for(int k = 0; k < 3; k++) { iv.minIDir[k] = iv.maxIDir[k] = 0.0f; iv.minOrg[k] = iv.maxOrg[k] = org[k][0]; }
	const int signBits = __builtin_amdgcn_readfirstlane((Q.d[0][0] < 0.0f ? 1 : 0) | (Q.d[1][0] < 0.0f ? 2 : 0) | (Q.d[2][0] < 0.0f ? 4 : 0));
	float tidBits[4];
#pragma unroll
	for(int l = 0; l < 4; l++) tidBits[l] = __int_as_float(tid[l]);
	const int sign16 = PACK ? signBits : signBits << 16;
	const u64 nodeBase = (u64)nodes;
	float stkN = __int_as_float(PACK ? (int)((unsigned)(size - 1) << 26) | 1 : 0), stkF = __int_as_float((size - 1) << 8);
	int sp = 1, first = 0, last = size - 1, cnt = 0;
	for(;;) {
		int leafSub, leafAux, sCur, sFl, sOff, sWidth;
		u64 sRng, sAlive;
		float vt[17];
		if(PACK) {
			int sTopw;
			if(COH) {
				if(SHADOW && REL) { SNAIL_DESCEND_PF2_OCT(SNAIL_PRE_NONE_X, SNAIL_ORG_SHARED, SNAIL_SLAB_COH_R, SNAIL_TAIL_ANY, "", SNAIL_COUNT, SNAIL_PF_LEAFREQ_SLOT0, oct) }
				else if(SHADOW) { SNAIL_DESCEND_PF2_OCT(SNAIL_PRE_SHARED, SNAIL_ORG_SHARED, SNAIL_SLAB_COH, SNAIL_TAIL_ANY, "", SNAIL_COUNT, SNAIL_PF_LEAFREQ_TRI, oct) }
				else if(POSDIST) { SNAIL_DESCEND_PF2_OCT(SNAIL_PRE_NONE_X, SNAIL_ORG_SHARED, SNAIL_SLAB_COH_R, SNAIL_TAIL_POS, SNAIL_COUNT, "", SNAIL_PF_LEAFREQ_SLOT0, oct) }
				else { SNAIL_DESCEND_PF2_OCT(SNAIL_PRE_SHARED, SNAIL_ORG_SHARED, SNAIL_SLAB_COH, SNAIL_TAIL_ANY, SNAIL_COUNT, "", SNAIL_PF_LEAFREQ_TRI, oct) }
			} else {
				if(SHADOW && REL) { SNAIL_DESCEND_PF2_PLAIN(SNAIL_PRE_NONE_X, SNAIL_ORG_SHARED, SNAIL_SLAB_FAST_R, SNAIL_TAIL_ANY, "", SNAIL_COUNT, SNAIL_PF_LEAFREQ_SLOT0); }
				else if(SHADOW) { SNAIL_DESCEND_PF2_PLAIN(SNAIL_PRE_SHARED, SNAIL_ORG_SHARED, SNAIL_SLAB_FAST, SNAIL_TAIL_ANY, "", SNAIL_COUNT, SNAIL_PF_LEAFREQ_TRI); }
				else if(POSDIST) { SNAIL_DESCEND_PF2_PLAIN(SNAIL_PRE_NONE_X, SNAIL_ORG_SHARED, SNAIL_SLAB_FAST_R, SNAIL_TAIL_POS, SNAIL_COUNT, "", SNAIL_PF_LEAFREQ_SLOT0); }
				else { SNAIL_DESCEND_PF2_PLAIN(SNAIL_PRE_SHARED, SNAIL_ORG_SHARED, SNAIL_SLAB_FAST, SNAIL_TAIL_ANY, SNAIL_COUNT, "", SNAIL_PF_LEAFREQ_TRI); }
			}
		} else if(COH) {
			if(SHADOW) { SNAIL_DESCEND_OCT(SNAIL_PRE_SHARED, SNAIL_ORG_SHARED, SNAIL_SLAB_COH, SNAIL_TAIL_ANY, "", SNAIL_COUNT, oct) }
			else if(POSDIST) { SNAIL_DESCEND_OCT(SNAIL_PRE_SHARED, SNAIL_ORG_SHARED, SNAIL_SLAB_COH, SNAIL_TAIL_POS, SNAIL_COUNT, "", oct) }
			else { SNAIL_DESCEND_OCT(SNAIL_PRE_SHARED, SNAIL_ORG_SHARED, SNAIL_SLAB_COH, SNAIL_TAIL_ANY, SNAIL_COUNT, "", oct) }
		} else {
			if(SHADOW) { SNAIL_DESCEND_ASM(SNAIL_PRE_SHARED, SNAIL_ORG_SHARED, SNAIL_SLAB_FAST, SNAIL_TAIL_ANY, "", SNAIL_COUNT, "s84", "s87", "s85", "s88", "s86", "s89"); }
			else if(POSDIST) { SNAIL_DESCEND_ASM(SNAIL_PRE_SHARED, SNAIL_ORG_SHARED, SNAIL_SLAB_FAST, SNAIL_TAIL_POS, SNAIL_COUNT, "", "s84", "s87", "s85", "s88", "s86", "s89"); }
			else { SNAIL_DESCEND_ASM(SNAIL_PRE_SHARED, SNAIL_ORG_SHARED, SNAIL_SLAB_FAST, SNAIL_TAIL_ANY, SNAIL_COUNT, "", "s84", "s87", "s85", "s88", "s86", "s89"); }
		}
		if(leafSub == 0) break;
		if(leafShared<MASK, SHADOW, COH ? M_COH : M_FAST, BARY>(tris, leafAux, (int)((unsigned)leafSub & 0x7fffffffu), size, lane, first, last, org, Q, mask4,
																 tidBits, bu, bv, iv, st))
			break;
	}
#pragma unroll
	for(int l = 0; l < 4; l++) tid[l] = __float_as_int(tidBits[l]);
	st.iters += SHADOW ? (unsigned)cnt : 2u * (unsigned)cnt - 1u;
}

template <bool MASK, bool COH, bool BARY, bool PACK>
__device__ __forceinline__ void walkPerRayAsm(const uint4 *__restrict__ nodes , const uint4 *__restrict__ tris, int size, int lane, const float (&org)[3][4],
											  Quad &Q, unsigned mask4, int (&tid)[4], float (&bu)[4], float (&bv)[4], Counters &st, const int oct) {
	const int signBits = __builtin_amdgcn_readfirstlane((Q.d[0][0] < 0.0f ? 1 : 0) | (Q.d[1][0] < 0.0f ? 2 : 0) | (Q.d[2][0] < 0.0f ? 4 : 0));
	const int sign16 = PACK ? (COH ? signBits | __builtin_amdgcn_readfirstlane(oct) << 8 : signBits) : signBits << 16;
	const u64 nodeBase = (u64)nodes;
	float stkN = __int_as_float(PACK ? (int)((unsigned)(size - 1) << 26) | 1 : 0), stkF = __int_as_float((size - 1) << 8);
	int sp = 1, first = 0, last = size - 1, cnt = 0;
	for(;;) {
		int leafSub, leafAux, sCur, sFl, sOff, sWidth;
		u64 sRng, sAlive;
		float vt[17];
		if(PACK) {
			int sTopw;
			if(COH) { SNAIL_DESCEND_PF2_SEL(SNAIL_ORG_PERRAY, SNAIL_SLABO_SEL, SNAIL_TAIL_ANY, SNAIL_COUNT, "", SNAIL_PF_LEAFREQ_TRI); }
			else { SNAIL_DESCEND_PF2_PLAIN(SNAIL_PRE_NONE, SNAIL_ORG_PERRAY, SNAIL_SLABO_FAST, SNAIL_TAIL_ANY, SNAIL_COUNT, "", SNAIL_PF_LEAFREQ_TRI); }
		} else if(COH) { SNAIL_DESCEND_OCT(SNAIL_PRE_NONE, SNAIL_ORG_PERRAY, SNAIL_SLABO_COH, SNAIL_TAIL_ANY, SNAIL_COUNT, "", oct) }
		else { SNAIL_DESCEND_ASM(SNAIL_PRE_NONE, SNAIL_ORG_PERRAY, SNAIL_SLABO_FAST, SNAIL_TAIL_ANY, SNAIL_COUNT, "", "s84", "s87", "s85", "s88", "s86", "s89"); }
		if(leafSub == 0) break;
		leafPerRay<MASK, COH ? M_COH : M_FAST, BARY>(tris, leafAux, (int)((unsigned)leafSub & 0x7fffffffu), lane, first, last, org, Q, mask4, tid, bu, bv, st);
	}
	st.iters += 2u * (unsigned)cnt - 1u;
}

__device__ __forceinline__ void finalBarycentrics(const uint4 *__restrict__ tris, const float (&org)[3][4], const Quad &Q, const int (&tid)[4],
												  float (&bu)[4], float (&bv)[4]) {
#if SNAIL_ARITH_SSE
	float det[4], uu[4], vv[4], idet[4];
#pragma unroll
	for(int l = 0; l < 4; l++) {
		det[l] = 1.0f; uu[l] = 0.0f; vv[l] = 0.0f;
		if(Q.dist[l] < __builtin_inff()) {
			const Tri t = loadTriVector(tris, tid[l]);
			const TriTerms tt = triTerms(t, org[0][0], org[1][0], org[2][0]);
			det[l] = Q.d[0][l] * t.n[0] + Q.d[1][l] * t.n[1] + Q.d[2][l] * t.n[2];
			vv[l] = Q.d[0][l] * tt.t0v[0] + Q.d[1][l] * tt.t0v[1] + Q.d[2][l] * tt.t0v[2];
			uu[l] = Q.d[0][l] * tt.t1v[0] + Q.d[1][l] * tt.t1v[1] + Q.d[2][l] * tt.t1v[2];
		}
	}
	InvN<4>(det, idet);
#pragma unroll
	for(int l = 0; l < 4; l++) {
		const bool hit = Q.dist[l] < __builtin_inff();
		bu[l] = hit ? uu[l] * idet[l] : 0.0f; bv[l] = hit ? vv[l] * idet[l] : 0.0f;
	}
#else
#pragma unroll
	for(int l = 0; l < 4; l++) {
		bu[l] = 0.0f; bv[l] = 0.0f;
		if(Q.dist[l] < __builtin_inff()) {
			const Tri t = loadTriVector(tris, tid[l]);
			const TriTerms tt = triTerms(t, org[0][0], org[1][0], org[2][0]);
			const float det = Q.d[0][l] * t.n[0] + Q.d[1][l] * t.n[1] + Q.d[2][l] * t.n[2];
			const float v = Q.d[0][l] * tt.t0v[0] + Q.d[1][l] * tt.t0v[1] + Q.d[2][l] * tt.t0v[2];
			const float u = Q.d[0][l] * tt.t1v[0] + Q.d[1][l] * tt.t1v[1] + Q.d[2][l] * tt.t1v[2];
			const float idet = Inv(det);
			bu[l] = u * idet; bv[l] = v * idet;
		}
	}
#endif
}

__device__ __forceinline__ int classify(bool fastOK, bool laneFinite, bool live, const float (&id)[3][4], const float (&dist)[4], int &oct) {
	oct = 0;
	if(!(fastOK && __all(laneFinite || !live))) return M_EXACT;
	bool coh = true;
#pragma unroll
	for(int k = 0; k < 3; k++) {
		bool anyNeg = false, anyPos = false;
#pragma unroll
		for(int l = 0; l < 4; l++) {
			const bool matters = dist[l] > -__builtin_inff();
			anyNeg |= matters && __float_as_int(id[k][l]) < 0;
			anyPos |= matters && __float_as_int(id[k][l]) >= 0;
		}
		const bool n = __any(anyNeg && live), p = __any(anyPos && live);
		coh = coh && !(n && p);
		oct |= n ? (1 << k) : 0;
	}
	return coh ? M_COH : M_FAST;
}

__device__ __forceinline__ bool originSaneDev(const float (&o)[3]) {
	return __builtin_fabsf(o[0]) <= 1.0e9f && __builtin_fabsf(o[1]) <= 1.0e9f && __builtin_fabsf(o[2]) <= 1.0e9f;
}
__device__ __forceinline__ bool finite4(const float (&v)[3][4]) {
	bool f = true;
#pragma unroll
	for(int c = 0; c < 3; c++)
#pragma unroll
		for(int l = 0; l < 4; l++) f = f && (__builtin_fabsf(v[c][l]) < __builtin_inff());
	return f;
}

__device__ __forceinline__ void flushStats(u64 *stats, const Counters &st, unsigned rays, int lane) {
	if(stats && lane == 0) {
		atomicAdd(&stats[0], (u64)st.intersects);
		atomicAdd(&stats[1], (u64)st.iters);
		atomicAdd(&stats[2], (u64)rays);
		atomicAdd(&stats[3], (u64)st.skips);
	}
}
__device__ __forceinline__ void bookPacket(unsigned *pstats, size_t packet, const Counters &st, unsigned rays, int lane) {
	if(pstats && lane == 0) {
		unsigned *w = pstats + packet * 4;
		atomicAdd(&w[0], st.intersects);
		atomicAdd(&w[1], st.iters);
		atomicAdd(&w[2], rays);
		atomicAdd(&w[3], st.skips);
	}
}

__device__ __forceinline__ int convChannelW(float c) {
	float v = c * 255.0f;
	v = v > 0.0f ? v : 0.0f;
	v = v < 255.0f ? v : 255.0f;
	return (int)v;
}

template <class ARGS>
__device__ __forceinline__ void bookPacketLate(size_t packet, const Counters &st, unsigned rays, int lane) {
	const ARGS __attribute__((address_space(4))) *E = (const ARGS __attribute__((address_space(4))) *)__builtin_amdgcn_kernarg_segment_ptr();
	asm volatile("" : "+s"(E));
	bookPacket(E->pstats, packet, st, rays, lane);
}

struct GenConst {
// ... 1173 lines not shown
	const int p = (int)blockIdx.x * 4 + (int)(threadIdx.x >> 6);
	if(p >= A.nPackets) return;
	const int2 xy = A.packetXY[p];
	const int yy = xy.y + (lane >> 2), xx = xy.x + (lane & 3) * 4;
	if(yy >= A.resy) return;
	const size_t src = (size_t)p * 256 + (size_t)lane * 4, dst = (size_t)yy * A.resx + xx;
#pragma unroll
	for(int l = 0; l < 4; l++)
		if(xx + l < A.resx) {
			if(A.t && A.pt) A.t[dst + l] = A.pt[src + l];
			if(A.u && A.pu) A.u[dst + l] = A.pu[src + l];
			if(A.v && A.pv) A.v[dst + l] = A.pv[src + l];
			if(A.id && A.pid) A.id[dst + l] = A.pid[src + l];
		}
}

#endif
__device__ __forceinline__ int convChannel(float c) {
	float v = c * 255.0f;
	v = v > 0.0f ? v : 0.0f;
	v = v < 255.0f ? v : 255.0f;
	return (int)v;
}
__global__ __launch_bounds__(256) void k_shade_depth(const unsigned *tables , const float *t, int nRays, unsigned char *bgr) {
	const int i = (int)(blockIdx.x * 256 + threadIdx.x) * 4;
	if(i >= nRays) return;
	const float4 tv = *(const float4 *)(t + i);
	const float tt[4] = {tv.x, tv.y, tv.z, tv.w};
	unsigned bytes[12];
#pragma unroll
	for(int l = 0; l < 4; l++) {
		const float dist = InvDiv(tt[l]);
		bytes[l * 3 + 0] = (unsigned)convChannel(dist * 2.0f); bytes[l * 3 + 1] = (unsigned)convChannel(dist * 250.0f); bytes[l * 3 + 2] = (unsigned)convChannel(dist * 20.0f);
	}
	if(((unsigned long long)bgr & 3) == 0) {
		unsigned *o = (unsigned *)(bgr + (size_t)i * 3);
#pragma unroll
		for(int k = 0; k < 3; k++) o[k] = bytes[4 * k] | (bytes[4 * k + 1] << 8) | (bytes[4 * k + 2] << 16) | (bytes[4 * k + 3] << 24);
	} else {
#pragma unroll
		for(int k = 0; k < 12; k++) bgr[(size_t)i * 3 + k] = (unsigned char)bytes[k];
	}
}
#if !SNAIL_ARITH_SSE
__global__ __launch_bounds__(256) void k_bgr_to_frame(const int2 *packetXY, int nPackets, int resx, int resy, const unsigned char *src,
														unsigned char *frame, int pitch, int nPerChunk, long long chunkStride) {
	const int lane = threadIdx.x & 63;
	const int p = (int)blockIdx.x * 4 + (int)(threadIdx.x >> 6);
	if(p >= nPackets) return;
	const int2 xy = packetXY[p];
	const int yy = xy.y + (lane >> 2), xx = xy.x + (lane & 3) * 4;
	if(yy >= resy) return;
	const unsigned char *s = nPerChunk > 0 ? src + (size_t)(p / nPerChunk) * (size_t)chunkStride + ((size_t)(p % nPerChunk) * 256 + (size_t)lane * 4) * 3
										   : src + ((size_t)p * 256 + (size_t)lane * 4) * 3;
	unsigned char *d = frame + (size_t)yy * pitch + (size_t)xx * 3;
	if(xx + 3 < resx && (pitch & 3) == 0 && (((unsigned long long)frame | (unsigned long long)src) & 3) == 0) {
		const unsigned *sw = (const unsigned *)s;
		unsigned *dw = (unsigned *)d;
		const unsigned a = sw[0], b = sw[1], c = sw[2];
		dw[0] = a; dw[1] = b; dw[2] = c;
		return;
	}
	for(int l = 0; l < 4; l++)
		if(xx + l < resx) { d[l * 3 + 0] = s[l * 3 + 0]; d[l * 3 + 1] = s[l * 3 + 1]; d[l * 3 + 2] = s[l * 3 + 2]; }
}

__global__ __launch_bounds__(256) void k_bgr_to_planar(const int4 *tiles, const int *firstPacket, const long long *outOff, int nTiles,
														 const unsigned char *src, unsigned char *out) {
	const int tile = (int)blockIdx.y;
	if(tile >= nTiles) return;
	const int4 T = tiles[tile];
	const int n = T.z * T.w;
	const int ppr = (T.z + 15) >> 4;
	unsigned char *o = out + outOff[tile];
	for(int i = (int)(blockIdx.x * blockDim.x + threadIdx.x); i < n; i += (int)(gridDim.x * blockDim.x)) {
		const int ty = i / T.z, tx = i - ty * T.z;
		const size_t pk = (size_t)firstPacket[tile] + (size_t)(ty >> 4) * ppr + (size_t)(tx >> 4);
		const unsigned char *s = src + (pk * 256 + (size_t)((ty & 15) * 16 + (tx & 15))) * 3;
		const unsigned char b = s[0], g = s[1], r = s[2];
		o[i] = r; o[(size_t)n + i] = (unsigned char)(g - r); o[(size_t)2 * n + i] = (unsigned char)(b - r);
	}
}
__global__ __launch_bounds__(256) void k_planar_to_frame(const int4 *tiles, const long long *inOff, int nTiles, const unsigned char *in, unsigned char *frame,
														   int pitch, int resx, int resy) {
	const int tile = (int)blockIdx.y;
	if(tile >= nTiles) return;
	const int4 T = tiles[tile];
	const int n = T.z * T.w;
	const unsigned char *p = in + inOff[tile];
	for(int i = (int)(blockIdx.x * blockDim.x + threadIdx.x); i < n; i += (int)(gridDim.x * blockDim.x)) {
		const int ty = i / T.z, tx = i - ty * T.z;
		const int xx = T.x + tx, yy = T.y + ty;
		if(xx >= resx || yy >= resy) continue;
		const unsigned char red = p[i];
		unsigned char *d = frame + (size_t)yy * pitch + (size_t)xx * 3;
		d[2] = red; d[1] = (unsigned char)(p[(size_t)n + i] + red); d[0] = (unsigned char)(p[(size_t)2 * n + i] + red);
	}
}

#ifdef SNAIL_DEBUG_API
__global__ __launch_bounds__(64) void k_delay(unsigned ticks) {
	const u64 t0 = __builtin_amdgcn_s_memrealtime();
	while((unsigned)(__builtin_amdgcn_s_memrealtime() - t0) < ticks) __builtin_amdgcn_s_sleep(1);
}

__global__ __launch_bounds__(64) void k_clock(unsigned ticks, unsigned long long *out) {
	const u64 r0 = __builtin_amdgcn_s_memrealtime(), c0 = __builtin_amdgcn_s_memtime();
	while((unsigned)(__builtin_amdgcn_s_memrealtime() - r0) < ticks) __builtin_amdgcn_s_sleep(1);
	const u64 c1 = __builtin_amdgcn_s_memtime(), r1 = __builtin_amdgcn_s_memrealtime();
	if(threadIdx.x == 0) { out[0] = c1 - c0; out[1] = r1 - r0; }
}

__global__ __launch_bounds__(256) void k_recip_check(unsigned base, unsigned long long *out) {
	const unsigned bits = base + blockIdx.x * 256u + threadIdx.x;
	const float x = __uint_as_float(bits);
	const float ref = 1.0f / x, got = recipExact(x);
	const bool same = (ref != ref) ? (got != got) : __float_as_uint(ref) == __float_as_uint(got);
	const bool inside = ((bits & 0x7f800000u) - 0x00800000u) < 0x7e000000u;
	const u64 bad = __builtin_amdgcn_ballot_w64(!same), in = __builtin_amdgcn_ballot_w64(inside);
	if((threadIdx.x & 63) == 0) {
		if(bad) atomicAdd(&out[0], (unsigned long long)__builtin_popcountll(bad));
		if(in) atomicAdd(&out[1], (unsigned long long)__builtin_popcountll(in));
	}
}

__global__ void k_nop(int *sink) { if(sink && threadIdx.x == 0 && blockIdx.x == 0x7fffffff) *sink = 1; }
#endif

__host__ __device__ inline void pfEncode(const unsigned (&in)[8], unsigned (&out)[8], unsigned trisOff) {
	for(int k = 0; k < 6; k++) out[k] = in[k];
	if(in[6] & 0x80000000u) { out[6] = 0x80000000u | (trisOff + ((in[6] & 0x7fffffffu) << 6)); out[7] = in[7]; }
	else { out[6] = (in[6] + 1u + (in[7] >> 16)) << 5; out[7] = 1u << (in[7] & 3u); }
}
__global__ __launch_bounds__(256) void k_pf_encode(const uint4 *__restrict__ nodes, int nNodes, unsigned trisOff, uint4 *__restrict__ pf) {
	const int i = (int)(blockIdx.x * 256 + threadIdx.x);
	if(i >= nNodes) return;
	const uint4 a = nodes[(size_t)i * 2], b = nodes[(size_t)i * 2 + 1];
	const unsigned in[8] = {a.x, a.y, a.z, a.w, b.x, b.y, b.z, b.w};
	unsigned out[8];
	pfEncode(in, out, trisOff);
	pf[(size_t)(i + 1) * 2] = make_uint4(out[0], out[1], out[2], out[3]);
	pf[(size_t)(i + 1) * 2 + 1] = make_uint4(out[4], out[5], out[6], out[7]);
}

__host__ __device__ inline bool relOriginInside(const unsigned (&w)[6]) {
	bool in = true;
	for(int k = 0; k < 3; k++) {
		const float n = __builtin_bit_cast(float, w[k]), f = __builtin_bit_cast(float, w[3 + k]);
		in = in && n <= 0.0f && f >= 0.0f;
	}
	return in;
}
__host__ __device__ inline unsigned relAux(const unsigned (&rel)[6], unsigned sub, unsigned aux) {
	return !(sub & 0x80000000u) && (aux & 7u) && relOriginInside(rel) ? aux | (1u << SNAIL_REL_INSIDE_BIT) : aux;
}
__global__ __launch_bounds__(256) void k_rel_nodes(const uint4 *__restrict__ pf, int nSlots, float ox, float oy, float oz, uint4 *__restrict__ rel) {
	const int i = (int)(blockIdx.x * 256 + threadIdx.x);
	if(i >= nSlots) return;
	const uint4 a = pf[(size_t)i * 2], b = pf[(size_t)i * 2 + 1];
	const float o[3] = {ox, oy, oz};
	const unsigned in[6] = {a.x, a.y, a.z, a.w, b.x, b.y};
	unsigned out[6];
	for(int k = 0; k < 6; k++) out[k] = __float_as_uint(__uint_as_float(in[k]) - o[k % 3]);
	rel[(size_t)i * 2] = make_uint4(out[0], out[1], out[2], out[3]);
	rel[(size_t)i * 2 + 1] = make_uint4(out[4], out[5], b.z, relAux(out, b.z, b.w));
}

struct RelFillArgs {
	int n;
	float org[SNAIL_MAX_BATCH][3];
	uint4 *dst[SNAIL_MAX_BATCH];
};
__global__ __launch_bounds__(256) void k_rel_nodes_multi(const uint4 *__restrict__ pf, int nSlots, RelFillArgs A) {
	const int i = (int)(blockIdx.x * 256 + threadIdx.x);
	if(i >= nSlots) return;
	const uint4 a = pf[(size_t)i * 2], b = pf[(size_t)i * 2 + 1];
	const unsigned in[6] = {a.x, a.y, a.z, a.w, b.x, b.y};
	for(int f = 0; f < A.n; f++) {
		unsigned out[6];
		for(int k = 0; k < 6; k++) out[k] = __float_as_uint(__uint_as_float(in[k]) - A.org[f][k % 3]);
		A.dst[f][(size_t)i * 2] = make_uint4(out[0], out[1], out[2], out[3]);
		A.dst[f][(size_t)i * 2 + 1] = make_uint4(out[4], out[5], b.z, relAux(out, b.z, b.w));
	}
}
#ifdef SNAIL_DEBUG_API
__global__ __launch_bounds__(256) void k_rel_flag_count(const uint4 *__restrict__ rel, int nSlots, unsigned long long *__restrict__ out) {
	const int i = (int)(blockIdx.x * 256 + threadIdx.x);
	const bool flagged = i < nSlots && !(rel[(size_t)i * 2 + 1].z & 0x80000000u) && ((rel[(size_t)i * 2 + 1].w >> SNAIL_REL_INSIDE_BIT) & 1u);
	const u64 m = __builtin_amdgcn_ballot_w64(flagged);
	if((threadIdx.x & 63) == 0 && m) atomicAdd(out, (unsigned long long)__builtin_popcountll(m));
}
#endif

struct AccountArgs {
	const uint4 *nodes, *tris;
	GenConst g;
	int x0, y0, pw, ph;
	u64 *out;
};
__global__ __launch_bounds__(256) void k_account(AccountArgs A) {
	const int lane = threadIdx.x & 63;
	const int p = (int)blockIdx.x * 4 + (int)(threadIdx.x >> 6);
	if(p >= A.pw * A.ph) return;
	const int px = A.x0 + (p % A.pw) * 16, py = A.y0 + (p / A.pw) * 16;
	const int ty = lane >> 2, k4 = lane & 3;
	const float inf = __builtin_inff();
	unsigned vn = 0, vt = 0, hits = 0;
	for(int l = 0; l < 4; l++) {
		const float xoff = (float)(px + (l >= 2 ? 2 : 0)), yoff = (float)(py - (l >= 2 ? 1 : 0));
		const float tposx = (float)(4 * k4) + xoff, tposy = (float)ty + yoff;
		float pp[3], d[3], id[3];
		for(int c = 0; c < 3; c++) pp[c] = A.g.tright[c] * tposx + (A.g.tup[c] * tposy + A.g.txyz[c][l]);
		const float rs = 1.0f / __builtin_sqrtf(pp[0] * pp[0] + pp[1] * pp[1] + pp[2] * pp[2]);
		for(int c = 0; c < 3; c++) { d[c] = pp[c] * rs; id[c] = 1.0f / (d[c] + 0.00000001f); }
		const int sg[3] = {d[0] < 0.0f, d[1] < 0.0f, d[2] < 0.0f};
		int stack[SNAIL_MAX_DEPTH + 2], sp = 0;
		stack[sp++] = 0;
		float dist = inf;
		while(sp) {
			int cur = stack[--sp];
			for(;;) {
				const uint4 *np = A.nodes + (size_t)cur * 2;
				const uint4 a = np[0], b = np[1];
				const float bmin[3] = {asf(a.x), asf(a.y), asf(a.z)}, bmax[3] = {asf(a.w), asf(b.x), asf(b.y)};
				vn++;
				float lmin = 0.0f, lmax = 0.0f;
				for(int k = 0; k < 3; k++) {
					float l1 = id[k] * (bmin[k] - A.g.org[k]), l2 = id[k] * (bmax[k] - A.g.org[k]);
					float lo = Min<M_EXACT>(l1, l2), hi = Max<M_EXACT>(l1, l2);
					if(k == 0) { lmin = lo; lmax = hi; }
					else { lmin = Max<M_EXACT>(lmin, lo); lmax = Min<M_EXACT>(lmax, hi); }
				}
				if(lmax < 0.0f || lmin > Min<M_EXACT>(lmax, dist)) break;
				if(b.z & 0x80000000u) {
					const int count = (int)b.w, firstTri = (int)(b.z & 0x7fffffffu);
					for(int k = 0; k < count; k++) {
						const Tri t = loadTriVector(A.tris, firstTri + k);
						vt++;
						float tv[3] = {A.g.org[0] - t.a[0], A.g.org[1] - t.a[1], A.g.org[2] - t.a[2]};
						float t0v[3] = {(t.ba[1] * tv[2] - t.ba[2] * tv[1]) * t.it0, (t.ba[2] * tv[0] - t.ba[0] * tv[2]) * t.it0,
										(t.ba[0] * tv[1] - t.ba[1] * tv[0]) * t.it0};
						float t1v[3] = {(tv[1] * t.ca[2] - tv[2] * t.ca[1]) * t.it0, (tv[2] * t.ca[0] - tv[0] * t.ca[2]) * t.it0,
										(tv[0] * t.ca[1] - tv[1] * t.ca[0]) * t.it0};
						const float tmul = -(tv[0] * t.n[0] + tv[1] * t.n[1] + tv[2] * t.n[2]);
						const float det = d[0] * t.n[0] + d[1] * t.n[1] + d[2] * t.n[2];
						const float v = d[0] * t0v[0] + d[1] * t0v[1] + d[2] * t0v[2];
						const float u = d[0] * t1v[0] + d[1] * t1v[1] + d[2] * t1v[2];
						const float duv = det - u - v;
						const float uvmin = Min<M_EXACT>(u, Min<M_EXACT>(v, duv)), uvmax = Max<M_EXACT>(u, Max<M_EXACT>(v, duv));
						if(!(uvmax <= 0.0f || uvmin >= 0.0f)) continue;
						const float t2 = (1.0f / det) * tmul;
						if(t2 < dist && t2 > 0.0f) dist = t2;
					}
					break;
				}
				const int child = (int)b.z, axis = (int)(b.w & 0xffff), fn = (int)((b.w >> 16) & 0xffff) ^ sg[axis];
				stack[sp++] = child + (fn ^ 1);
				cur = child + fn;
			}
		}
		if(dist < inf) hits++;
	}
	u64 r0 = 4, r1 = vn, r2 = vt, r3 = hits;
	for(int o = 32; o > 0; o >>= 1) {
		r0 += __shfl_xor(r0, o); r1 += __shfl_xor(r1, o); r2 += __shfl_xor(r2, o); r3 += __shfl_xor(r3, o);
	}
	if(lane == 0) { atomicAdd(&A.out[0], r0); atomicAdd(&A.out[1], r1); atomicAdd(&A.out[2], r2); atomicAdd(&A.out[3], r3); }
}

#endif
}
```

snail_amd/csrc/snail_hip.hip:

```cpp
#include <hip/hip_runtime.h>
#include <hip/hip_ext.h>

#include <cmath>
#include <cstdarg>
#include <cstdio>
#include <algorithm>
#include <cstring>
#include <memory>
#include <mutex>
#include <utility>
#include <vector>

#include "../../include/snail_hip.h"
#include "../../include/snail_instances.h"
#include "../../include/snail_bvh_fast.h"
#include "host_sse.h"
#ifdef SNAIL_DEBUG_API
#include "../../include/snail_hip_debug.h"
#endif

static thread_local char g_err[1024] = "";

void snail_set_error(const char *fmt, ...) {
	va_list ap;
// ... 505 lines not shown
	HIP_TRY(hipMemset(W.defer, 0, 16 * sizeof(int)));
	HIP_TRY(hipDeviceSynchronize());
	W.sDist = (float *)base; base += rays * 4 * SNAIL_MAX_LIGHTS;
	W.pstats = (unsigned *)base; base += packets * 16;
	W.heatXY = (int *)base; base += packets * 16;
	if(refl) {
		W.rOrg = (float *)base; base += quads * 48;
		W.rDir = (float *)base; base += quads * 48;
		W.rIDir = (float *)base; base += quads * 48;
		W.rDist = (float *)base; base += rays * 4;
		W.rObj = (int *)base; base += rays * 4;
		W.rCol = (float *)base; base += rays * 12;
		W.rMask = (unsigned char *)base;
	}
	return 0;
}

template <bool SHARED, bool MASK>
void launchRaysKernels(const SnailScene *s, const dev::RaysArgs &A, int blocks, const ExactPass &EP, hipStream_t stream) {
	const bool deep = useDeep(s), bary = A.bary != nullptr, sse = s->arith == SNAIL_ARITH_HOST_SSE;
#define SNAIL_RAYS_LAUNCH(D, B)                                                                                                            \
	do {                                                                                                                                   \
		SNAIL_LAUNCH(sse, RaysArgs, dim3(blocks), dim3(64), 0, stream, A, k_rays<SHARED, MASK, D, B>);                                      \
		SNAIL_LAUNCH(sse, RaysArgs, EP.grid, EP.block, EP.lds, stream, A, k_rays_exact<SHARED, MASK, D, B>);                                \
	} while(0)
	if(deep && bary) SNAIL_RAYS_LAUNCH(true, true);
	else if(deep) SNAIL_RAYS_LAUNCH(true, false);
	else if(bary) SNAIL_RAYS_LAUNCH(false, true);
	else SNAIL_RAYS_LAUNCH(false, false);
#undef SNAIL_RAYS_LAUNCH
}

int launchRays(SnailScene *s, bool shadow, int nPackets, int size, int sharedOrigin, const float *origin, const float *dir,
					  const float *idir, const uint8_t *mask, float *distance, int32_t *object, float *bary, uint64_t *dStats, hipStream_t stream,
					  const int32_t *dOrder = nullptr, int32_t *dSlotCost = nullptr, int nSlots = 0, int32_t *dNextOrder = nullptr, int orderFlags = 0,
					  uint32_t *dPacketStats = nullptr) {
	if(nPackets <= 0) return 0;
	if(size < 1 || size > SNAIL_PACKET_QUADS) { snail_set_error("packet size %d outside 1..%d quads", size, SNAIL_PACKET_QUADS); return 1; }
	if(!origin || !dir || !idir || !distance || (!shadow && !object)) { snail_set_error("null ray array"); return 1; }
	SceneUse use(s, stream);
	if(use.rc) return use.rc;
	dev::RaysArgs A;
	memset(&A, 0, sizeof(A));
	A.hostTab = s->arith == SNAIL_ARITH_HOST_SSE ? s->dTab : nullptr;
	A.nodes = s->dNodes; A.tris = s->dTris; A.pf = (const uint4 *)s->dPF;
	A.nPackets = nPackets; A.size = size; A.fastOK = s->fastOK; A.pack = stackPack(s);
	A.origin = origin; A.dir = dir; A.idir = idir; A.mask = mask;
	A.distance = distance; A.object = object; A.bary = bary;
	A.stats = (dev::u64 *)dStats;
	A.pstats = shadow ? nullptr : dPacketStats;
	int blocks = ((nPackets + 127) / 128) * 128;
	if(!shadow && (dOrder || dSlotCost) && nSlots >= nPackets) {
		A.order = dOrder; A.slotCost = dSlotCost; A.nSlots = nSlots;
		if(nSlots > blocks) blocks = ((nSlots + 127) / 128) * 128;
	}
	SnailScene::RayDefer &R = s->rayDefer[s->rayCount++ % SnailScene::kDeferSlots];
	if((size_t)nPackets + 16 > R.cap) {
		HIP_TRY(hipDeviceSynchronize());
		if(R.p) (void)hipFree(R.p);
		R.p = nullptr; R.cap = 0;
		HIP_TRY(hipMalloc((void **)&R.p, ((size_t)nPackets + 16) * sizeof(int)));
		HIP_TRY(hipMemset(R.p, 0, 16 * sizeof(int)));
		HIP_TRY(hipDeviceSynchronize());
		R.cap = (size_t)nPackets + 16;
	}
	if(!R.done) HIP_TRY(hipEventCreateWithFlags(&R.done, hipEventDisableTiming));
	if(R.used) HIP_TRY(hipStreamWaitEvent(stream, R.done, 0));
	A.defer = R.p;
	const int exactBlocks = A.fastOK ? (blocks < 8 ? blocks : 8) : (blocks < 2048 ? blocks : 2048);
	const ExactPass EP = exactPassFor(exactBlocks, A.slotCost, A.nSlots, shadow ? nullptr : dNextOrder, orderFlags);
	A.nextOrder = EP.nextOrder; A.nextOrderFlags = EP.orderFlags;
	if(shadow) {
		if(useDeep(s)) {
			hipLaunchKernelGGL(dev::k_shadow<true>, dim3(blocks), dim3(64), 0, stream, A);
			hipLaunchKernelGGL(dev::k_shadow_exact<true>, dim3(exactBlocks), dim3(64), 0, stream, A);
		} else {
			hipLaunchKernelGGL(dev::k_shadow<false>, dim3(blocks), dim3(64), 0, stream, A);
			hipLaunchKernelGGL(dev::k_shadow_exact<false>, dim3(exactBlocks), dim3(64), 0, stream, A);
		}
	} else if(A.pstats) {
		if(sharedOrigin || !mask || bary) { snail_set_error("per-packet counters: mirrored packets only"); return 1; }
		const bool sse = s->arith == SNAIL_ARITH_HOST_SSE;
		if(useDeep(s)) {
			SNAIL_LAUNCH(sse, RaysArgs, dim3(blocks), dim3(64), 0, stream, A, k_rays<false, true, true, false, true>);
			SNAIL_LAUNCH(sse, RaysArgs, EP.grid, EP.block, EP.lds, stream, A, k_rays_exact<false, true, true, false, true>);
		} else {
			SNAIL_LAUNCH(sse, RaysArgs, dim3(blocks), dim3(64), 0, stream, A, k_rays<false, true, false, false, true>);
			SNAIL_LAUNCH(sse, RaysArgs, EP.grid, EP.block, EP.lds, stream, A, k_rays_exact<false, true, false, false, true>);
		}
	} else if(sharedOrigin && mask) launchRaysKernels<true, true>(s, A, blocks, EP, stream);
	else if(sharedOrigin) launchRaysKernels<true, false>(s, A, blocks, EP, stream);
	else if(mask) launchRaysKernels<false, true>(s, A, blocks, EP, stream);
	else launchRaysKernels<false, false>(s, A, blocks, EP, stream);
	HIP_TRY(hipGetLastError());
	if(EP.sortAfter) { if(int rc = snail_order_from_cost_hint_dev(A.slotCost, A.nSlots, dNextOrder, EP.orderFlags, stream)) return rc; }
	HIP_TRY(hipEventRecord(R.done, stream));
	R.used = true;
	return 0;
}

template <int SRC>
int launchLights(SnailScene *s, dev::ShadeArgs A , hipStream_t stream, int32_t *dNextOrder = nullptr, int orderFlags = 0) {
	if(A.nLights <= 0) return 0;
	SceneUse use(s, stream);
	if(use.rc) return use.rc;
	int relWhich[SNAIL_MAX_LIGHTS];
	for(int n = 0; n < SNAIL_MAX_LIGHTS; n++) { relWhich[n] = -1; A.relLight[n] = nullptr; }
	if(A.pack && !useDeep(s))
		for(int n = 0; n < A.nLights; n++)
			if(int rc = relFor(s, A.lights[n], stream, &A.relLight[n], &relWhich[n])) return rc;
	const dim3 grid(A.nBlocks, A.nLights);
	const int total = A.nBlocks * A.nLights;
	const int exactBlocks = A.fastOK ? (total < 8 ? total : 8) : (total < 2048 ? total : 2048);
	const bool sse = s->arith == SNAIL_ARITH_HOST_SSE;
	const ExactPass EP = exactPassFor(exactBlocks, A.slotCost, A.nSlots, dNextOrder, orderFlags);
	A.nextOrder = EP.nextOrder; A.nextOrderFlags = EP.orderFlags;
	if(A.pstats) {
		if(useDeep(s)) {
			SNAIL_LAUNCH(sse, ShadeArgs, grid, dim3(64), 0, stream, A, k_light<true, SRC, true>);
			SNAIL_LAUNCH(sse, ShadeArgs, EP.grid, EP.block, EP.lds, stream, A, k_light_exact<true, SRC, true>);
		} else {
			SNAIL_LAUNCH(sse, ShadeArgs, grid, dim3(64), 0, stream, A, k_light<false, SRC, true>);
			SNAIL_LAUNCH(sse, ShadeArgs, EP.grid, EP.block, EP.lds, stream, A, k_light_exact<false, SRC, true>);
		}
	} else if(useDeep(s)) {
		SNAIL_LAUNCH(sse, ShadeArgs, grid, dim3(64), 0, stream, A, k_light<true, SRC>);
		SNAIL_LAUNCH(sse, ShadeArgs, EP.grid, EP.block, EP.lds, stream, A, k_light_exact<true, SRC>);
	} else {
		SNAIL_LAUNCH(sse, ShadeArgs, grid, dim3(64), 0, stream, A, k_light<false, SRC>);
		SNAIL_LAUNCH(sse, ShadeArgs, EP.grid, EP.block, EP.lds, stream, A, k_light_exact<false, SRC>);
	}
	HIP_TRY(hipGetLastError());
	if(EP.sortAfter) { if(int rc = snail_order_from_cost_hint_dev(A.slotCost, A.nSlots, dNextOrder, EP.orderFlags, stream)) return rc; }
	for(int n = 0; n < A.nLights; n++)
		if(relWhich[n] >= 0) { if(int rc = relUsed(s, relWhich[n], stream)) return rc; }
	return 0;
}

}

#include "lbvh.inc"

extern "C" {

const char *snail_last_error(void) { return g_err; }

int snail_device_count(void) {
	int n = 0;
	if(hipGetDeviceCount(&n) != hipSuccess) return 0;
	return n;
}

static size_t pfTrisOffset(int) { return (size_t)1 << 25; }

SnailScene *snail_scene_create(const void *nodes32, int nNodes, const void *tris64, int nTris, int depth, int device) {
	if(!nodes32 || !tris64 || nNodes <= 0 || nTris <= 0) { snail_set_error("snail_scene_create: empty scene"); return nullptr; }
	if(depth < 0 || depth > SNAIL_MAX_DEPTH) { snail_set_error("snail_scene_create: depth %d outside 0..BVH::maxDepth = %d", depth, SNAIL_MAX_DEPTH); return nullptr; }
	const uint32_t *nw = (const uint32_t *)nodes32;
	int pairsOdd = 1;
	for(int i = 0; i < nNodes; i++) {
		uint32_t sub = nw[i * 8 + 6], aux = nw[i * 8 + 7];
		if(sub & 0x80000000u) {
			uint32_t first = sub & 0x7fffffffu;
			if((int32_t)aux < 0 || (uint64_t)first + aux > (uint64_t)nTris) { snail_set_error("snail_scene_create: leaf %d references triangles [%u,%u) of %d", i, first, first + aux, nTris); return nullptr; }
		} else {
			if((uint64_t)sub + 1 >= (uint64_t)nNodes || sub == 0) { snail_set_error("snail_scene_create: node %d has child %u of %d", i, sub, nNodes); return nullptr; }
			if((aux & 0xffff) > 2 || (aux >> 16) > 1) { snail_set_error("snail_scene_create: node %d has axis/firstNode %u/%u", i, aux & 0xffff, aux >> 16); return nullptr; }
			if(!(sub & 1u)) pairsOdd = 0;
		}
	}
	int realDepth = 0, nestedOK = 1;
	{
		std::vector<uint8_t> seen((size_t)nNodes, 0);
		std::vector<std::pair<int, int>> todo;
		todo.emplace_back(0, 0);
		while(!todo.empty()) {
			const auto [i, level] = todo.back();
			todo.pop_back();
			if(seen[i]) { snail_set_error("snail_scene_create: node %d is reachable twice from the root (cycle or shared subtree)", i); return nullptr; }
			seen[i] = 1;
			if(level > realDepth) realDepth = level;
			if(level > depth) { snail_set_error("snail_scene_create: node %d lies at level %d, deeper than the declared depth %d", i, level, depth); return nullptr; }
			const uint32_t sub = nw[(size_t)i * 8 + 6];
			if(!(sub & 0x80000000u)) {
				todo.emplace_back((int)sub + 1, level + 1); todo.emplace_back((int)sub, level + 1);
				const float *pb = (const float *)nodes32 + (size_t)i * 8;
				for(int c = 0; c < 2; c++) {
					const float *cb = (const float *)nodes32 + ((size_t)sub + c) * 8;
					for(int k = 0; k < 3; k++)
						if(!(cb[k] >= pb[k]) || !(cb[3 + k] <= pb[3 + k])) nestedOK = 0;
				}
			}
		}
	}
	int fastOK = 1;
	const float *tf = (const float *)tris64;
	for(int i = 0; i < nTris && fastOK; i++) {
		const float *r = tf + (size_t)i * 16;
		for(int k = 0; k < 9; k++) if(!(std::fabs(r[k]) <= 1.0e9f)) fastOK = 0;
		if(!(r[9] > 0.0f) || !(r[10] <= 1.0e12f) || !(r[10] > 0.0f)) fastOK = 0;
		for(int k = 12; k < 16; k++) if(!(std::fabs(r[k]) <= 1.0e18f)) fastOK = 0;
	}
	const float *nf = (const float *)nodes32;
	for(int i = 0; i < nNodes && fastOK; i++) {
		for(int k = 0; k < 6; k++) if(!(std::fabs(nf[(size_t)i * 8 + k]) <= 1.0e9f)) fastOK = 0;
		for(int k = 0; k < 3; k++) if(!(nf[(size_t)i * 8 + k] <= nf[(size_t)i * 8 + 3 + k])) fastOK = 0;
	}

	DeviceGuard guard(device);
	if(!guard.ok) { snail_set_error("snail_scene_create: hipSetDevice(%d) failed", device); return nullptr; }
	SnailScene *s = new SnailScene();
	s->device = device; s->nNodes = nNodes; s->nTris = nTris; s->depth = realDepth; s->fastOK = fastOK; s->nestedOK = nestedOK;
	const size_t trisOff = pfTrisOffset(nNodes), pfBytes = trisOff + (size_t)nTris * 64;
	const bool fits = (size_t)nNodes + 1 < ((size_t)1 << 20) && pfBytes < ((size_t)1 << 31);
	s->pfOKButNesting = pairsOdd && fits;
	s->pfOK = s->pfOKButNesting && nestedOK;
	s->trisOff = (int)(fits ? trisOff : 0);
	std::vector<uint32_t> pf;
	if(s->pfOKButNesting) {
		pf.assign(((size_t)nNodes + 1) * 8, 0u);
		for(int i = 0; i < nNodes; i++) {
			unsigned in[8], out[8];
			for(int k = 0; k < 8; k++) in[k] = nw[(size_t)i * 8 + k];
			dev::pfEncode(in, out, (unsigned)trisOff);
			for(int k = 0; k < 8; k++) pf[((size_t)i + 1) * 8 + k] = out[k];
		}
	}
	hipError_t e;
	if((e = hipMalloc((void **)&s->dNodes, (size_t)nNodes * 32)) != hipSuccess || (e = hipMalloc((void **)&s->dPF, fits ? pfBytes : (size_t)nTris * 64)) != hipSuccess ||
	   (e = hipMemcpy(s->dNodes, nodes32, (size_t)nNodes * 32, hipMemcpyHostToDevice)) != hipSuccess ||
	   (e = hipMemcpy(s->dPF + s->trisOff, tris64, (size_t)nTris * 64, hipMemcpyHostToDevice)) != hipSuccess ||
	   (!pf.empty() && (e = hipMemcpy(s->dPF, pf.data(), pf.size() * 4, hipMemcpyHostToDevice)) != hipSuccess)) {
		snail_set_error("snail_scene_create: %s", hipGetErrorString(e));
		snail_scene_destroy(s);
		return nullptr;
	}
	s->dTris = (uint4 *)(s->dPF + s->trisOff);
	return s;
}

SnailScene *snail_scene_create_lbvh(const float *tri_verts, int nTris, int device, int maxLeafTris, int32_t *perm, float *build_ms) {
	if(!tri_verts || nTris <= 0 || maxLeafTris < 1 || maxLeafTris > 64) { snail_set_error("snail_scene_create_lbvh: bad arguments (1 <= maxLeafTris <= 64)"); return nullptr; }
	DeviceGuard guard(device);
	if(!guard.ok) { snail_set_error("snail_scene_create_lbvh: hipSetDevice(%d) failed", device); return nullptr; }
	uint4 *dNodes = nullptr, *dTris = nullptr;
	int depth = 0, fastOK = 0;
	if(buildLbvhDevice(tri_verts, nTris, maxLeafTris, &dNodes, &dTris, perm, &depth, &fastOK, build_ms)) return nullptr;
	if(depth > SNAIL_MAX_DEPTH) {
		(void)hipFree(dNodes); (void)hipFree(dTris);
		snail_set_error("snail_scene_create_lbvh: depth %d exceeds BVH::maxDepth %d", depth, SNAIL_MAX_DEPTH);
		return nullptr;
	}
	SnailScene *s = new SnailScene();
	s->device = device; s->nNodes = 2 * nTris - 1; s->nTris = nTris; s->depth = depth; s->fastOK = fastOK;
	s->dNodes = dNodes;
	const size_t trisOff = pfTrisOffset(s->nNodes), pfBytes = trisOff + (size_t)nTris * 64;
	const bool fits = (size_t)s->nNodes + 1 < ((size_t)1 << 20) && pfBytes < ((size_t)1 << 31);
	s->trisOff = (int)(fits ? trisOff : 0);
	s->nestedOK = 1; s->pfOKButNesting = s->pfOK = fits ? 1 : 0;
	hipError_t e;
	if((e = hipMalloc((void **)&s->dPF, fits ? pfBytes : (size_t)nTris * 64)) != hipSuccess ||
	   (e = hipMemcpy(s->dPF + s->trisOff, dTris, (size_t)nTris * 64, hipMemcpyDeviceToDevice)) != hipSuccess) {
		(void)hipFree(dTris);
		snail_set_error("snail_scene_create_lbvh: %s", hipGetErrorString(e));
		snail_scene_destroy(s);
		return nullptr;
	}
	(void)hipFree(dTris);
	s->dTris = (uint4 *)(s->dPF + s->trisOff);
	if(fits) {
		(void)hipMemset(s->dPF, 0, 32);
		hipLaunchKernelGGL(dev::k_pf_encode, dim3((unsigned)((s->nNodes + 255) / 256)), dim3(256), 0, 0, s->dNodes, s->nNodes, (unsigned)trisOff, (uint4 *)s->dPF);
		if((e = hipDeviceSynchronize()) != hipSuccess) {
			snail_set_error("snail_scene_create_lbvh: %s", hipGetErrorString(e));
			snail_scene_destroy(s);
			return nullptr;
		}
	}
	return s;
}

int snail_scene_download(const SnailScene *s, void *nodes32, void *tris64) {
	if(int rc = checkScene(s, "snail_scene_download")) return rc;
	DeviceGuard guard(s->device);
	int nNodes = s->nNodes;
	if(s->fast) {
		int cur[4];
		if(int rc = fastCurrent(s, cur)) return rc;
		nNodes = cur[0];
	}
	if(nodes32) HIP_TRY(hipMemcpy(nodes32, s->dNodes, (size_t)nNodes * 32, hipMemcpyDeviceToHost));
	if(tris64) HIP_TRY(hipMemcpy(tris64, s->dTris, (size_t)s->nTris * 64, hipMemcpyDeviceToHost));
	return 0;
}

void snail_scene_destroy(SnailScene *s) {
	if(!s) return;
	DeviceGuard guard(s->device);
	freeTileJobs(s);
	if(s->dNodes) (void)hipFree(s->dNodes);
	if(s->dPF) (void)hipFree(s->dPF);
	if(s->dTab) (void)hipFree(s->dTab);
	fastFree(s->fast);
	for(auto &e : s->rel) {
		if(e.d) (void)hipFree(e.d);
		if(e.filled) (void)hipEventDestroy(e.filled);
		for(hipEvent_t ev : e.used) if(ev) (void)hipEventDestroy(ev);
	}
	for(SnailScene::HostCall *c : s->hostFree) {
		if(c->arena) (void)hipFree(c->arena);
		if(c->dStats) (void)hipFree(c->dStats);
		if(c->stream) (void)hipStreamDestroy(c->stream);
		delete c;
	}
	for(int k = 0; k < SnailScene::kDeferSlots; k++) if(s->dDefer[k]) (void)hipFree(s->dDefer[k]);
	for(int k = 0; k < SnailScene::kDeferSlots; k++) if(s->shade[k].hitT) (void)hipFree(s->shade[k].hitT);
	for(int k = 0; k < SnailScene::kDeferSlots; k++) {
		if(s->rayDefer[k].p) (void)hipFree(s->rayDefer[k].p);
		if(s->rayDefer[k].done) (void)hipEventDestroy(s->rayDefer[k].done);
		if(s->deferDone[k]) (void)hipEventDestroy(s->deferDone[k]);
		if(s->shade[k].done) (void)hipEventDestroy(s->shade[k].done);
	}
	delete s;
}

int snail_scene_info(const SnailScene *s, int *nNodes, int *nTris, int *depth, int *device) {
	if(!s) { snail_set_error("snail_scene_info: null scene"); return 1; }
	int cur[4] = {s->nNodes, s->depth, 0, 0};
	if(s->fast) { if(int rc = fastCurrent(s, cur)) return rc; }
	if(nNodes) *nNodes = cur[0];
	if(nTris) *nTris = s->nTris;
	if(depth) *depth = cur[1];
	if(device) *device = s->device;
	return 0;
}

int snail_scene_flags(const SnailScene *s, int *fastOK, int *nestedOK) {
	if(!s) { snail_set_error("snail_scene_flags: null scene"); return 1; }
	if(fastOK) *fastOK = s->fastOK;
	if(nestedOK) *nestedOK = s->nestedOK;
	return 0;
}

int snail_scene_set_arith(SnailScene *s, int arith) {
	if(int rc = checkScene(s, "snail_scene_set_arith")) return rc;
	if(arith != SNAIL_ARITH_IEEE && arith != SNAIL_ARITH_HOST_SSE) { snail_set_error("snail_scene_set_arith: unknown arithmetic %d", arith); return 1; }
	SNAIL_LOCK(s);
	if(arith == SNAIL_ARITH_HOST_SSE) {
		DeviceGuard guard(s->device);
		if(!guard.ok) { snail_set_error("snail_scene_set_arith: hipSetDevice(%d) failed", s->device); return 1; }
		if(int rc = hostSseFill("snail_scene_set_arith", &s->dTab, &s->tabGen)) return rc;
	}
	s->arith = arith;
	return 0;
}
int snail_scene_arith(const SnailScene *s, int *arith) {
	if(int rc = checkScene(s, "snail_scene_arith")) return rc;
	if(arith) *arith = s->arith;
	return 0;
}
int snail_arith_set_tables(const uint32_t *tables12288) {
	const char *why = "";
	if(hostSseSetTables(tables12288, &why)) { snail_set_error("snail_arith_set_tables: %s", why); return 1; }
	return 0;
}
int snail_arith_prepare_device(void) {
	const unsigned *tab = nullptr;
	return hostSseDeviceTables("snail_arith_prepare_device", &tab);
}
int snail_host_sse_tables(uint32_t *tables12288) {
	const char *why = "";
	if(hostSseSnapshot((unsigned *)tables12288, nullptr, &why)) { snail_set_error("snail_host_sse_tables: %s", why); return 2; }
	return 0;
}
int snail_host_sse_check(int fn, uint64_t first, uint64_t count, int threads, uint64_t *mismatches, uint32_t *firstBad) {
	if((fn != 0 && fn != 1) || first > (1ull << 32) || count > (1ull << 32) - first || !mismatches) { snail_set_error("snail_host_sse_check: bad arguments"); return 1; }
	const char *why = "";
	if(hostSseSnapshot(nullptr, nullptr, &why)) { snail_set_error("snail_host_sse_check: %s", why); return 2; }
	unsigned bad = 0;
	*mismatches = hostSseMismatches(fn, first, count, threads, &bad);
	if(firstBad) *firstBad = bad;
	return 0;
}

int snail_last_launch(const SnailScene *s, int *blocks, int *threads) {
	if(!s) { snail_set_error("snail_last_launch: null scene"); return 1; }
	std::lock_guard<std::mutex> lock(const_cast<SnailScene *>(s)->mu);
	if(blocks) *blocks = s->lastBlocks;
	if(threads) *threads = s->lastThreads;
	return 0;
}

int snail_trace_primary_dev(SnailScene *s, const float cam[13], int resx, int resy, int x0, int y0, int w, int h, float *t, float *u,
							float *v, int32_t *id, uint64_t *dStats, void *stream) {
	if(int rc = checkScene(s, "snail_trace_primary_dev")) return rc;
	DeviceGuard guard(s->device);
	SNAIL_LOCK(s);
	return launchPrimary(s, cam, resx, resy, x0, y0, w, h, nullptr, 0, t, u, v, id, dStats, (hipStream_t)stream);
}

int snail_primary_slots(int w, int h) {
	if(w <= 0 || h <= 0) return 0;
	const int pw = (w + 15) / 16, ph = (h + 15) / 16;
	return (((pw + 3) / 4) * ((ph + 3) / 4) + 7) / 8 * 8 * 16;
}

int snail_trace_primary_ordered_dev(SnailScene *s, const float cam[13], int resx, int resy, int x0, int y0, int w, int h, float *t, float *u,
									float *v, int32_t *id, uint64_t *dStats, const int32_t *dOrder, int32_t *dSlotCost, void *stream) {
	if(int rc = checkScene(s, "snail_trace_primary_ordered_dev")) return rc;
	DeviceGuard guard(s->device);
// ... 482 lines not shown
	HIP_TRY(hipGetLastError());
	return 0;
}

#ifdef SNAIL_DEBUG_API
int snail_debug_delay_dev(float microseconds, void *stream) {
	if(!(microseconds >= 0.0f) || microseconds > 10000.0f) { snail_set_error("snail_debug_delay_dev: delay outside 0..10000 us"); return 1; }
	const unsigned ticks = (unsigned)(microseconds * 100.0f);
	if(ticks == 0) return 0;
	hipLaunchKernelGGL(dev::k_delay, dim3(1), dim3(64), 0, (hipStream_t)stream, ticks);
	HIP_TRY(hipGetLastError());
	return 0;
}

int snail_debug_clock_dev(float microseconds, uint64_t *dOut2, void *stream) {
	if(!(microseconds > 0.0f) || microseconds > 10000.0f || !dOut2) { snail_set_error("snail_debug_clock_dev: bad arguments"); return 1; }
	hipLaunchKernelGGL(dev::k_clock, dim3(1), dim3(64), 0, (hipStream_t)stream, (unsigned)(microseconds * 100.0f), (unsigned long long *)dOut2);
	HIP_TRY(hipGetLastError());
	return 0;
}

int snail_debug_recip_check(uint64_t out2[2]) {
	if(!out2) { snail_set_error("snail_debug_recip_check: bad arguments"); return 1; }
	unsigned long long *d = nullptr;
	HIP_TRY(hipMalloc(&d, 16));
	HIP_TRY(hipMemset(d, 0, 16));
	for(unsigned part = 0; part < 256; part++) hipLaunchKernelGGL(dev::k_recip_check, dim3(1u << 16), dim3(256), 0, 0, part << 24, d);
	hipError_t e = hipDeviceSynchronize();
	if(e == hipSuccess) e = hipMemcpy(out2, d, 16, hipMemcpyDeviceToHost);
	(void)hipFree(d);
	HIP_TRY(e);
	return 0;
}

int snail_debug_hostsse_device_check(int fn, int threads, uint64_t *badChunks, uint32_t *firstBadChunk) {
	if((fn != 0 && fn != 1) || !badChunks) { snail_set_error("snail_debug_hostsse_device_check: bad arguments"); return 1; }
	const unsigned *tab = nullptr;
	if(int rc = hostSseDeviceTables("snail_debug_hostsse_device_check", &tab)) return rc;
	constexpr unsigned kBatch = 4096;
	unsigned long long *d = nullptr;
	HIP_TRY(hipMalloc((void **)&d, kBatch * sizeof(unsigned long long)));
	std::vector<unsigned long long> got(kBatch), want(kBatch);
	uint64_t bad = 0;
	uint32_t first = 0xffffffffu;
	for(unsigned c0 = 0; c0 < 65536u; c0 += kBatch) {
		hipError_t e = hipMemset(d, 0, kBatch * sizeof(unsigned long long));
		if(e == hipSuccess) { hipLaunchKernelGGL(dev_sse::k_hostsse_sums, dim3(kBatch), dim3(256), 0, 0, tab, fn, c0, d); e = hipGetLastError(); }
		hostSseChunkSums(fn, c0, kBatch, threads, want.data());
		if(e == hipSuccess) e = hipMemcpy(got.data(), d, kBatch * sizeof(unsigned long long), hipMemcpyDeviceToHost);
		if(e != hipSuccess) { (void)hipFree(d); snail_set_error("snail_debug_hostsse_device_check: %s", hipGetErrorString(e)); return 100 + (int)e; }
		for(unsigned k = 0; k < kBatch; k++)
			if(got[k] != want[k]) { if(!bad) first = c0 + k; bad++; }
	}
	(void)hipFree(d);
	*badChunks = bad;
	if(firstBadChunk) *firstBadChunk = first;
	return 0;
}

int snail_debug_dispatch_rate(int blocks, int threads, int reps, float *ms_per_launch) {
	if(blocks <= 0 || threads <= 0 || threads > 1024 || reps <= 0 || !ms_per_launch) { snail_set_error("snail_debug_dispatch_rate: bad arguments"); return 1; }
	hipEvent_t e0, e1;
	HIP_TRY(hipEventCreate(&e0)); HIP_TRY(hipEventCreate(&e1));
	hipLaunchKernelGGL(dev::k_nop, dim3(blocks), dim3(threads), 0, 0, (int *)nullptr);
	HIP_TRY(hipDeviceSynchronize());
	HIP_TRY(hipEventRecord(e0, 0));
	for(int r = 0; r < reps; r++) hipLaunchKernelGGL(dev::k_nop, dim3(blocks), dim3(threads), 0, 0, (int *)nullptr);
	HIP_TRY(hipEventRecord(e1, 0));
	HIP_TRY(hipDeviceSynchronize());
	float ms = 0.0f;
	HIP_TRY(hipEventElapsedTime(&ms, e0, e1));
	(void)hipEventDestroy(e0); (void)hipEventDestroy(e1);
	*ms_per_launch = ms / reps;
	return 0;
}

int snail_debug_anyorder(SnailScene *s, const float cam[13], int resx, int resy, int frames, int flags, float *ms_total) {
	if(int rc = checkScene(s, "snail_debug_anyorder")) return rc;
	if(frames <= 0 || !ms_total || useDeep(s)) { snail_set_error("snail_debug_anyorder: bad arguments"); return 1; }
	DeviceGuard guard(s->device);
	dev::PrimaryArgs A;
	memset(&A, 0, sizeof(A));
	A.hostTab = nullptr;
	A.nodes = s->dNodes; A.tris = s->dTris; A.pf = (const uint4 *)s->dPF;
	A.nFrames = 1;
	A.g[0] = makeGen(cam, resx, resy);
	A.resx = resx; A.resy = resy; A.w = resx; A.h = resy;
	A.fastOK = s->fastOK && originSane(cam);
	A.pack = stackPack(s);
	A.pw = (resx + 15) / 16; A.ph = (resy + 15) / 16; A.nPackets = A.pw * A.ph;
	const int nRegions = ((A.pw + 3) / 4) * ((A.ph + 3) / 4);
	const int blocks = ((nRegions + 7) / 8) * 8 * 16;
	A.nBlocks = blocks; A.nSlots = blocks;
	if(blocks + 2 > s->deferCap) { snail_set_error("snail_debug_anyorder: trace one ordinary frame of this size first"); return 1; }
	A.defer = s->dDefer[0];
	hipStream_t st;
	HIP_TRY(hipStreamCreateWithFlags(&st, hipStreamNonBlocking));
	int relWhich = -1;
	if(A.pack && !useDeep(s)) {
		if(int rc = relFor(s, cam, st, &A.rel[0], &relWhich)) return rc;
	}
	hipEvent_t e0, e1;
	HIP_TRY(hipEventCreate(&e0)); HIP_TRY(hipEventCreate(&e1));
	HIP_TRY(hipDeviceSynchronize());
	HIP_TRY(hipEventRecord(e0, st));
	for(int f = 0; f < frames; f++)
		hipExtLaunchKernelGGL(dev::k_primary<false>, dim3(blocks), dim3(64), 0, st, nullptr, nullptr, (unsigned)flags, A);
	HIP_TRY(hipGetLastError());
	HIP_TRY(hipEventRecord(e1, st));
	HIP_TRY(hipStreamSynchronize(st));
	HIP_TRY(hipEventElapsedTime(ms_total, e0, e1));
	(void)hipEventDestroy(e0); (void)hipEventDestroy(e1); (void)hipStreamDestroy(st);
	return 0;
}

int snail_debug_occupancy(int out[4]) {
	if(!out) { snail_set_error("snail_debug_occupancy: null output"); return 1; }
	int dev = 0;
	HIP_TRY(hipGetDevice(&dev));
	int perCU = 0, maxBlocks = 0, cus = 0;
	HIP_TRY(hipOccupancyMaxActiveBlocksPerMultiprocessor(&perCU, (const void *)dev::k_primary<false>, 64, 0));
	HIP_TRY(hipDeviceGetAttribute(&maxBlocks, hipDeviceAttributeMaxBlocksPerMultiProcessor, dev));
	HIP_TRY(hipDeviceGetAttribute(&cus, hipDeviceAttributeMultiprocessorCount, dev));
	out[0] = perCU; out[1] = maxBlocks; out[2] = cus; out[3] = 1;
	return 0;
}

int snail_debug_rel_flag_count(SnailScene *s, const float org[3], int *count) {
	if(int rc = checkScene(s, "snail_debug_rel_flag_count")) return rc;
	if(!org || !count) { snail_set_error("snail_debug_rel_flag_count: null argument"); return 1; }
	if(!stackPack(s)) { snail_set_error("snail_debug_rel_flag_count: this scene keeps no origin-relative node records"); return 1; }
	DeviceGuard guard(s->device);
	HostCallScope hc(s, "snail_debug_rel_flag_count");
	if(hc.rc) return hc.rc;
	if(int rc = hc.zeroStats()) return rc;
	{
		SNAIL_LOCK(s);
		SceneUse use(s, hc.stream());
		if(use.rc) return use.rc;
		const uint4 *rel = nullptr;
		int which = -1;
		if(int rc = relFor(s, org, hc.stream(), &rel, &which)) return rc;
		const int nSlots = s->nNodes + 1;
		hipLaunchKernelGGL(dev::k_rel_flag_count, dim3((unsigned)((nSlots + 255) / 256)), dim3(256), 0, hc.stream(), rel, nSlots, (unsigned long long *)hc.stats());
		HIP_TRY(hipGetLastError());
		if(int rc = relUsed(s, which, hc.stream())) return rc;
	}
	uint64_t st[4] = {0, 0, 0, 0};
	if(int rc = hc.finish(st)) return rc;
	*count = (int)st[0];
	return 0;
}

#endif

int snail_account_packets(SnailScene *s, const float cam[13], int resx, int resy, uint32_t *out8) {
	if(int rc = checkScene(s, "snail_account_packets")) return rc;
	if(!out8 || resx <= 0 || resy <= 0) { snail_set_error("snail_account_packets: null output or bad resolution"); return 1; }
	DeviceGuard guard(s->device);
	HostCallScope hc(s, "snail_account_packets");
	if(hc.rc) return hc.rc;
	const size_t bytes = (size_t)((resx + 15) / 16) * ((resy + 15) / 16) * 32;
	if(int rc = hc.reserve(HostCallScope::pad(bytes))) return rc;
	void *c = hc.carve(bytes);
	HIP_TRY(hipMemsetAsync(c, 0, bytes, hc.stream()));
	{
		SNAIL_LOCK(s);
		if(int rc = launchPrimary(s, cam, resx, resy, 0, 0, resx, resy, nullptr, 0, nullptr, nullptr, nullptr, nullptr, nullptr, hc.stream(), (unsigned *)c)) return rc;
	}
	if(int rc = hc.get(out8, c, bytes)) return rc;
	return hc.finish(nullptr);
}

int snail_account_primary(SnailScene *s, const float cam[13], int resx, int resy, int x0, int y0, int w, int h, uint64_t out[4]) {
	if(int rc = checkScene(s, "snail_account_primary")) return rc;
	if((x0 & 15) || (y0 & 15) || w <= 0 || h <= 0 || !out) { snail_set_error("snail_account_primary: bad rect"); return 1; }
	DeviceGuard guard(s->device);
	HostCallScope hc(s, "snail_account_primary");
	if(hc.rc) return hc.rc;
	dev::AccountArgs A;
	A.nodes = s->dNodes; A.tris = s->dTris;
	A.g = makeGen(cam, resx, resy);
	A.x0 = x0; A.y0 = y0; A.pw = (w + 15) / 16; A.ph = (h + 15) / 16;
	A.out = (dev::u64 *)hc.stats();
	if(int rc = hc.zeroStats()) return rc;
	const int np = A.pw * A.ph;
	{
		SNAIL_LOCK(s);
		SceneUse use(s, hc.stream());
		if(use.rc) return use.rc;
		hipLaunchKernelGGL(dev::k_account, dim3((np + 3) / 4), dim3(256), 0, hc.stream(), A);
		HIP_TRY(hipGetLastError());
	}
	return hc.finish(out);
}

}

#include "bvh_fast.inc"
#include "render_host.inc"
#include "instances_host.inc"
#include "instances_tiles_host.inc"
#include "heatmap_host.inc"
#include "materials_host.inc"
#include "materials_tiles_host.inc"
```

Before: 27440 Mrays/s.

## Skip slab near-clamp for origin-relative nodes via per-axis sign bits in aux

Precomputes per-axis flags (near plane positive, far plane negative) into the aux word of origin-relative node records. The coherent POSDIST traversal then takes a fast path using a shorter slab tail that drops the max-with-zero clamp, whenever the node's octant mask bits are set. Otherwise it falls back to duplicated slow-path code copies. Leaf aux is masked to strip the new bits, and the fit check now limits triangle count to the 25-bit field. This adds code size and a scalar test per visit, and only affects the POSDIST coherent path.

Result: faster. 27960 Mrays/s, median of 6 (+1.9%).

```diff
diff --git a/include/snail_hip_debug.h b/include/snail_hip_debug.h
--- a/include/snail_hip_debug.h
+++ b/include/snail_hip_debug.h
@@ -21,6 +21,8 @@
 
 int snail_debug_rel_flag_count(SnailScene *, const float org[3], int *count);
 
+int snail_debug_rel_axis_flag_count(SnailScene *, const float org[3], int out[6]);
+
 #ifdef __cplusplus
 }
 #endif
diff --git a/snail_amd/_lib.py b/snail_amd/_lib.py
--- a/snail_amd/_lib.py
+++ b/snail_amd/_lib.py
@@ -152,6 +152,7 @@
     "snail_debug_occupancy": (_I, [_VP]),
     "snail_debug_anyorder": (_I, [_VP, _F13, _I, _I, _I, _I, _VP]),
     "snail_debug_rel_flag_count": (_I, [_VP, _VP, _VP]),
+    "snail_debug_rel_axis_flag_count": (_I, [_VP, _VP, _VP]),
 }
 DEBUG_LIB_PATH = os.path.join(HERE, "libsnailhip_debug.so")
 _dbg = None
diff --git a/snail_amd/csrc/bvh_fast.inc b/snail_amd/csrc/bvh_fast.inc
--- a/snail_amd/csrc/bvh_fast.inc
+++ b/snail_amd/csrc/bvh_fast.inc
@@ -189,7 +189,7 @@
 	const int cap = 2 * nTris - 1;
 	s->device = device; s->nNodes = cap; s->nTris = nTris;
 	const size_t trisOff = pfTrisOffset(cap), pfBytes = trisOff + (size_t)nTris * 64;
-	const bool fits = (size_t)cap + 1 < ((size_t)1 << 20) && pfBytes < ((size_t)1 << 31);
+	const bool fits = pfFits((size_t)cap + 1, (size_t)nTris);
 	s->trisOff = (int)(fits ? trisOff : 0);
 	s->pfOKButNesting = fits ? 1 : 0;
 	hipError_t e;
diff --git a/snail_amd/csrc/snail_dev.inc b/snail_amd/csrc/snail_dev.inc
--- a/snail_amd/csrc/snail_dev.inc
+++ b/snail_amd/csrc/snail_dev.inc
@@ -897,6 +897,7 @@
 		[oy2] "v"(org[1][2]), [oy3] "v"(org[1][3]), [oz0] "v"(org[2][0]), [oz1] "v"(org[2][1]), [oz2] "v"(org[2][2]), [oz3] "v"(org[2][3])
 #define SNAIL_TAIL_POS(L, S) "v_max_f32 %[t0], 0, %[t0]\n v_min_f32 %[t3], %[t3], %[d" L "]\n v_sub_f32 %[" S "], %[t3], %[t0]\n"
 #define SNAIL_TAIL_ANY(L, S) "v_min_f32 %[t4], %[t3], %[d" L "]\n v_sub_f32 %[t4], %[t4], %[t0]\n v_min_f32 %[" S "], %[t4], %[t3]\n"
+#define SNAIL_TAIL_POSF(L, S) "v_min_f32 %[t3], %[t3], %[d" L "]\n v_sub_f32 %[" S "], %[t3], %[t0]\n"
 #define SNAIL_POP_2W                                                                                                                       \
 	" v_readlane_b32 %[cur], %[stkN], %[sp]\n v_readlane_b32 %[fl], %[stkF], %[sp]\n"                                                      \
 	" s_and_b32 %[first], %[fl], 0xff\n s_lshr_b32 %[last], %[fl], 8\n"
@@ -971,8 +972,9 @@
 #define SNAIL_PF2_ALIVE " s_sub_u32 %[cur], %[last], %[first]\n s_bfm_b64 %[alive], %[cur], %[first]\n s_bitset1_b64 %[alive], %[last]\n"
 #define SNAIL_PF2_FIRSTLAST " s_ff1_i32_b64 %[first], exec\n s_flbit_i32_b64 %[last], exec\n s_xor_b32 %[last], %[last], 63\n"
 static_assert(SNAIL_REL_INSIDE_BIT == 31, "SNAIL_OIN_TEST_SNAIL_TAIL_POS names the bit in its text");
-#define SNAIL_OIN_TEST_SNAIL_TAIL_POS(AUX, LBL) " s_bitcmp1_b32 " AUX ", 31\n s_cbranch_scc1 " LBL "_%=\n"
-#define SNAIL_OIN_TEST_SNAIL_TAIL_ANY(AUX, LBL) ""
+#define SNAIL_OIN_TEST_SNAIL_TAIL_POS(AUX, CP, OMASK) " s_bitcmp1_b32 " AUX ", 31\n s_cbranch_scc1 L_oin" CP "_%=\n"
+#define SNAIL_OIN_TEST_SNAIL_TAIL_ANY(AUX, CP, OMASK) ""
+#define SNAIL_OIN_TEST_SNAIL_TAIL_POSF(AUX, CP, OMASK) " s_and_b32 vcc_lo, " AUX ", " OMASK "\n s_cbranch_scc0 L_slow" CP "_%=\n"
 #define SNAIL_OIN_TEST_of(TAIL) SNAIL_OIN_TEST_##TAIL
 #define SNAIL_OIN_PENDING(X, Y, OTHERSET, SUB, AUX, FARX, FARY, CNTVISIT, LEAFREQ)                                                          \
 				 "L_oin" X "p_%=:\n" CNTVISIT                                          \
@@ -993,12 +995,15 @@
 				 SNAIL_OIN_PENDING("B", "A", "s[84:91]", "s82", "s83", "%[width]", "%[fl]", CNTVISIT, LEAFREQ)                               \
 				 SNAIL_OIN_PENDING("A", "B", "s[76:83]", "s90", "s91", "%[fl]", "%[width]", CNTVISIT, LEAFREQ)
 #define SNAIL_OIN_COPIES_SNAIL_TAIL_ANY(CNTVISIT, LEAFREQ) ""
+#define SNAIL_OIN_COPIES_SNAIL_TAIL_POSF SNAIL_OIN_COPIES_SNAIL_TAIL_POS
 #define SNAIL_OIN_COPIES_of(TAIL) SNAIL_OIN_COPIES_##TAIL
-#define SNAIL_PF2_PENDING(X, OTHERSET, SUB, AUX, FARX, FARY, PRE, SLAB, TAIL, CNTVISIT, LEAFREQ, NX, FX, NY, FY, NZ, FZ)                                                   \
+#define SNAIL_PF2_PENDING(X, OTHERSET, SUB, AUX, FARX, FARY, PRE, SLAB, TAIL, CNTVISIT, LEAFREQ, OMASK, NX, FX, NY, FY, NZ, FZ)                                            \
 				 "L_visit" X "p_%=:\n"                                                                                                      \
 				 " s_waitcnt lgkmcnt(0)\n"                                                 \
 				 " s_load_dwordx8 s[68:75], %[base], " FARY "\n"                              \
-				 SNAIL_OIN_TEST_of(TAIL)(AUX, "L_oin" X "p")                                                                                  \
+				 SNAIL_OIN_TEST_of(TAIL)(AUX, X "p", OMASK)                                                                                   \
+				 SNAIL_PF2_PENDBODY(X, OTHERSET, SUB, AUX, FARX, FARY, PRE, SLAB, TAIL, CNTVISIT, LEAFREQ, NX, FX, NY, FY, NZ, FZ)
+#define SNAIL_PF2_PENDBODY(X, OTHERSET, SUB, AUX, FARX, FARY, PRE, SLAB, TAIL, CNTVISIT, LEAFREQ, NX, FX, NY, FY, NZ, FZ)                                                  \
 				 CNTVISIT PRE(NX, FX, NY, FY, NZ, FZ)                                                                                        \
 				 SLAB("0", NX, FX, NY, FY, NZ, FZ) TAIL("0", "s0")                                                                           \
 				 SNAIL_PF2_NEARFAR(SUB, AUX, FARX, OTHERSET, LEAFREQ)                                                                        \
@@ -1011,11 +1016,42 @@
 				 " v_writelane_b32 %[stkN], %[topw], m0\n s_add_u32 m0, m0, 1\n" SNAIL_PF2_ISLEAF(SUB)                                       \
 				 SLAB("3", NX, FX, NY, FY, NZ, FZ) TAIL("3", "s3")                                                                           \
 				 SNAIL_PF2_TAIL(X, SUB)
+#define SNAIL_PF2_POPBODY(PRE, SLAB, TAIL, CNTVISIT, LEAFREQ, NXA, FXA, NYA, FYA, NZA, FZA)                                                  \
+				 CNTVISIT PRE(NXA, FXA, NYA, FYA, NZA, FZA)                                                                                 \
+				 SLAB("0", NXA, FXA, NYA, FYA, NZA, FZA) TAIL("0", "s0")                                                          \
+				 " s_and_b32 %[cur], %[topw], 0xfffff\n s_lshl_b32 %[off], %[cur], 5\n"                                                    \
+				 " s_load_dwordx8 s[68:75], %[base], %[off]\n"                                                                             \
+				 SLAB("1", NXA, FXA, NYA, FYA, NZA, FZA) TAIL("1", "s1")                                                          \
+				 SNAIL_PF2_NEARFAR("s90", "s91", "%[fl]", "s[76:83]", LEAFREQ)                                                                       \
+				 SLAB("2", NXA, FXA, NYA, FYA, NZA, FZA) TAIL("2", "s2")                                                          \
+				 " s_bfe_u32 %[first], %[topw], 0x60014\n s_lshr_b32 %[last], %[topw], 26\n" SNAIL_PF2_ALIVE SNAIL_PF2_ISLEAF("s90")        \
+				 SLAB("3", NXA, FXA, NYA, FYA, NZA, FZA) TAIL("3", "s3")                                                          \
+				 SNAIL_PF2_TAIL("A", "s90")
+#define SNAIL_REL_NEARPOS_BIT 25
+#define SNAIL_REL_FARNEG_BIT 28
+#define SNAIL_REL_COUNT_MASK 0x01ffffffu
+static_assert(SNAIL_REL_NEARPOS_BIT == 25 && SNAIL_REL_FARNEG_BIT == 28 && SNAIL_REL_COUNT_MASK == (1u << SNAIL_REL_NEARPOS_BIT) - 1u,
+			  "SNAIL_DESCEND_PF2_OCT's masks and SNAIL_PF2_LEAF name the bits in their text");
+#define SNAIL_POSENTRY_PENDING(X, Y, OTHERSET, SUB, AUX, FARX, FARY, PRE, SLAB, CNTVISIT, LEAFREQ, NX, FX, NY, FY, NZ, FZ)                    \
+				 "L_slow" X "p_%=:\n"                                                   \
+				 SNAIL_OIN_TEST_SNAIL_TAIL_POS(AUX, X "p", "")                                                                               \
+				 SNAIL_PF2_PENDBODY(X, OTHERSET, SUB, AUX, FARX, FARY, PRE, SLAB, SNAIL_TAIL_POS, CNTVISIT, LEAFREQ, NX, FX, NY, FY, NZ, FZ)  \
+				 " s_branch L_visit" Y "p_%=\n"
+#define SNAIL_POSENTRY_COPIES_SNAIL_TAIL_POSF(PRE, SLAB, CNTVISIT, LEAFREQ, NXA, FXA, NYA, FYA, NZA, FZA, NXB, FXB, NYB, FYB, NZB, FZB)        \
+				 "L_slowAq_%=:\n"                                                         \
+				 SNAIL_OIN_TEST_SNAIL_TAIL_POS("s91", "Aq", "")                                                                              \
+				 SNAIL_PF2_POPBODY(PRE, SLAB, SNAIL_TAIL_POS, CNTVISIT, LEAFREQ, NXA, FXA, NYA, FYA, NZA, FZA)                               \
+				 " s_branch L_visitBp_%=\n"                                                                                                \
+				 SNAIL_POSENTRY_PENDING("B", "A", "s[84:91]", "s82", "s83", "%[width]", "%[fl]", PRE, SLAB, CNTVISIT, LEAFREQ, NXB, FXB, NYB, FYB, NZB, FZB) \
+				 SNAIL_POSENTRY_PENDING("A", "B", "s[76:83]", "s90", "s91", "%[fl]", "%[width]", PRE, SLAB, CNTVISIT, LEAFREQ, NXA, FXA, NYA, FYA, NZA, FZA)
+#define SNAIL_POSENTRY_COPIES_SNAIL_TAIL_POS(PRE, SLAB, CNTVISIT, LEAFREQ, NXA, FXA, NYA, FYA, NZA, FZA, NXB, FXB, NYB, FYB, NZB, FZB) ""
+#define SNAIL_POSENTRY_COPIES_SNAIL_TAIL_ANY(PRE, SLAB, CNTVISIT, LEAFREQ, NXA, FXA, NYA, FYA, NZA, FZA, NXB, FXB, NYB, FYB, NZB, FZB) ""
+#define SNAIL_POSENTRY_COPIES_of(TAIL) SNAIL_POSENTRY_COPIES_##TAIL
 #define SNAIL_PF2_LEAF(X, SUB, AUX)                                                                                                         \
 				 "L_leaf" X "_%=:\n" SNAIL_PF2_FIRSTLAST                                                                                    \
 				 " s_bfe_u32 %[leafSub], " SUB ", 0x190006\n s_sub_u32 %[leafSub], %[leafSub], 0x80000\n s_bitset1_b32 %[leafSub], 31\n"   \
-				 " s_mov_b32 %[leafAux], " AUX "\n s_waitcnt lgkmcnt(0)\n s_branch L_end_%=\n"
-#define SNAIL_DESCEND_PF2X(EXTRACLOB, PREVARS, PRE, ORGOPS, SLAB, TAIL, CNTPOP, CNTVISIT, LEAFREQ, NXA, FXA, NYA, FYA, NZA, FZA, NXB, FXB, NYB, FYB, NZB, FZB)                                                  \
+				 " s_and_b32 %[leafAux], " AUX ", 0x01ffffff\n s_waitcnt lgkmcnt(0)\n s_branch L_end_%=\n"
+#define SNAIL_DESCEND_PF2X(EXTRACLOB, OMASK, PREVARS, PRE, ORGOPS, SLAB, TAIL, CNTPOP, CNTVISIT, LEAFREQ, NXA, FXA, NYA, FYA, NZA, FZA, NXB, FXB, NYB, FYB, NZB, FZB)                                                  \
 	asm volatile(SNAIL_DRAIN_SMEM " s_mov_b32 m0, %[sp]\n"                                                                                \
 				 "L_entry_%=:\n"                                                                                                           \
 				 " s_cmp_eq_u32 m0, 0\n s_cbranch_scc1 L_done_%=\n"                                                                     \
@@ -1031,24 +1067,16 @@
 				                   \
 				 " s_sub_u32 %[off], m0, 1\n s_max_i32 %[off], %[off], 0\n"   \
 				 " v_readlane_b32 %[topw], %[stkN], %[off]\n"                                                                              \
-				 SNAIL_OIN_TEST_of(TAIL)("s91", "L_oinAq")                                                                                  \
-				 CNTVISIT PRE(NXA, FXA, NYA, FYA, NZA, FZA)                                                                                 \
-				 SLAB("0", NXA, FXA, NYA, FYA, NZA, FZA) TAIL("0", "s0")                                                          \
-				 " s_and_b32 %[cur], %[topw], 0xfffff\n s_lshl_b32 %[off], %[cur], 5\n"                                                    \
-				 " s_load_dwordx8 s[68:75], %[base], %[off]\n"                                                                             \
-				 SLAB("1", NXA, FXA, NYA, FYA, NZA, FZA) TAIL("1", "s1")                                                          \
-				 SNAIL_PF2_NEARFAR("s90", "s91", "%[fl]", "s[76:83]", LEAFREQ)                                                                       \
-				 SLAB("2", NXA, FXA, NYA, FYA, NZA, FZA) TAIL("2", "s2")                                                          \
-				 " s_bfe_u32 %[first], %[topw], 0x60014\n s_lshr_b32 %[last], %[topw], 26\n" SNAIL_PF2_ALIVE SNAIL_PF2_ISLEAF("s90")        \
-				 SLAB("3", NXA, FXA, NYA, FYA, NZA, FZA) TAIL("3", "s3")                                                          \
-				 SNAIL_PF2_TAIL("A", "s90")                                                                                                 \
+				 SNAIL_OIN_TEST_of(TAIL)("s91", "Aq", OMASK)                                                                                 \
+				 SNAIL_PF2_POPBODY(PRE, SLAB, TAIL, CNTVISIT, LEAFREQ, NXA, FXA, NYA, FYA, NZA, FZA)                                         \
 				                                                                    \
-				 SNAIL_PF2_PENDING("B", "s[84:91]", "s82", "s83", "%[width]", "%[fl]", PRE, SLAB, TAIL, CNTVISIT, LEAFREQ, NXB, FXB, NYB, FYB, NZB, FZB)                   \
+				 SNAIL_PF2_PENDING("B", "s[84:91]", "s82", "s83", "%[width]", "%[fl]", PRE, SLAB, TAIL, CNTVISIT, LEAFREQ, OMASK, NXB, FXB, NYB, FYB, NZB, FZB)            \
 				                                                                    \
-				 SNAIL_PF2_PENDING("A", "s[76:83]", "s90", "s91", "%[fl]", "%[width]", PRE, SLAB, TAIL, CNTVISIT, LEAFREQ, NXA, FXA, NYA, FYA, NZA, FZA)                   \
+				 SNAIL_PF2_PENDING("A", "s[76:83]", "s90", "s91", "%[fl]", "%[width]", PRE, SLAB, TAIL, CNTVISIT, LEAFREQ, OMASK, NXA, FXA, NYA, FYA, NZA, FZA)            \
 				 " s_branch L_visitBp_%=\n"                                                                                                \
 				 SNAIL_PF2_LEAF("A", "s90", "s91") SNAIL_PF2_LEAF("B", "s82", "s83")                                                       \
 				 SNAIL_OIN_COPIES_of(TAIL)(CNTVISIT, LEAFREQ)                                                                               \
+				 SNAIL_POSENTRY_COPIES_of(TAIL)(PRE, SLAB, CNTVISIT, LEAFREQ, NXA, FXA, NYA, FYA, NZA, FZA, NXB, FXB, NYB, FYB, NZB, FZB)    \
 				 "L_fail_%=:\n"                                                                                                            \
 				 " s_cmp_eq_u32 m0, 0\n s_cbranch_scc0 L_pop_%=\n"                                                                      \
 				 "L_done_%=:\n s_mov_b32 %[leafSub], 0\n s_mov_b32 %[leafAux], 0\n s_waitcnt lgkmcnt(0)\n"                                  \
@@ -1076,8 +1104,8 @@
 #define SNAIL_PRE_NONE_X(NX, FX, NY, FY, NZ, FZ) ""
 #define SNAIL_PREVARS_SNAIL_PRE_NONE_X SNAIL_PREVARS_EMPTY
 #define SNAIL_PREVARS_of(PRE) SNAIL_PREVARS_##PRE
-#define SNAIL_DESCEND_PF2(PRE, ORGOPS, SLAB, TAIL, CNTPOP, CNTVISIT, LEAFREQ, NXA, FXA, NYA, FYA, NZA, FZA, NXB, FXB, NYB, FYB, NZB, FZB)                 \
-	SNAIL_DESCEND_PF2X(, SNAIL_PREVARS_of(PRE), PRE, ORGOPS, SLAB, TAIL, CNTPOP, CNTVISIT, LEAFREQ, NXA, FXA, NYA, FYA, NZA, FZA, NXB, FXB, NYB, FYB, NZB, FZB)
+#define SNAIL_DESCEND_PF2M(OMASK, PRE, ORGOPS, SLAB, TAIL, CNTPOP, CNTVISIT, LEAFREQ, NXA, FXA, NYA, FYA, NZA, FZA, NXB, FXB, NYB, FYB, NZB, FZB)                 \
+	SNAIL_DESCEND_PF2X(, OMASK, SNAIL_PREVARS_of(PRE), PRE, ORGOPS, SLAB, TAIL, CNTPOP, CNTVISIT, LEAFREQ, NXA, FXA, NYA, FYA, NZA, FZA, NXB, FXB, NYB, FYB, NZB, FZB)
 #define SNAIL_PRE_SEL(NX, FX, NY, FY, NZ, FZ)                                                                                               \
 				 " s_bitcmp1_b32 %[sign16], 8\n s_cselect_b32 s62, " FX ", " NX "\n s_cselect_b32 s65, " NX ", " FX "\n"                       \
 				 " s_bitcmp1_b32 %[sign16], 9\n s_cselect_b32 s63, " FY ", " NY "\n s_cselect_b32 s66, " NY ", " FY "\n"                       \
@@ -1085,18 +1113,18 @@
 #define SNAIL_SLABO_SEL(L, NX, FX, NY, FY, NZ, FZ) SNAIL_SLABO_COH(L, "s62", "s65", "s63", "s66", "s64", "s67")
 #define SNAIL_SEL_CLOB , "s62", "s63", "s64", "s65", "s66", "s67"
 #define SNAIL_DESCEND_PF2_SEL(ORGOPS, SLAB, TAIL, CNTPOP, CNTVISIT, LEAFREQ)                                                                \
-	SNAIL_DESCEND_PF2X(SNAIL_SEL_CLOB, SNAIL_PREVARS_NONE, SNAIL_PRE_SEL, ORGOPS, SLAB, TAIL, CNTPOP, CNTVISIT, LEAFREQ, "s84", "s87", "s85", "s88", "s86", "s89", "s76", "s79", "s77", "s80", "s78", "s81")
-#define SNAIL_DESCEND_PF2_PLAIN(PRE, ORGOPS, SLAB, TAIL, CNTPOP, CNTVISIT, LEAFREQ) SNAIL_DESCEND_PF2(PRE, ORGOPS, SLAB, TAIL, CNTPOP, CNTVISIT, LEAFREQ, "s84", "s87", "s85", "s88", "s86", "s89", "s76", "s79", "s77", "s80", "s78", "s81")
+	SNAIL_DESCEND_PF2X(SNAIL_SEL_CLOB, "0", SNAIL_PREVARS_NONE, SNAIL_PRE_SEL, ORGOPS, SLAB, TAIL, CNTPOP, CNTVISIT, LEAFREQ, "s84", "s87", "s85", "s88", "s86", "s89", "s76", "s79", "s77", "s80", "s78", "s81")
+#define SNAIL_DESCEND_PF2_PLAIN(PRE, ORGOPS, SLAB, TAIL, CNTPOP, CNTVISIT, LEAFREQ) SNAIL_DESCEND_PF2M("0", PRE, ORGOPS, SLAB, TAIL, CNTPOP, CNTVISIT, LEAFREQ, "s84", "s87", "s85", "s88", "s86", "s89", "s76", "s79", "s77", "s80", "s78", "s81")
 #define SNAIL_DESCEND_PF2_OCT(PRE, ORGOPS, SLAB, TAIL, CNTPOP, CNTVISIT, LEAFREQ, OCT)                                                                                                    \
 	switch(OCT) {                                                                                                                          \
-	case 0: SNAIL_DESCEND_PF2(PRE, ORGOPS, SLAB, TAIL, CNTPOP, CNTVISIT, LEAFREQ, "s84", "s87", "s85", "s88", "s86", "s89", "s76", "s79", "s77", "s80", "s78", "s81"); break;            \
-	case 1: SNAIL_DESCEND_PF2(PRE, ORGOPS, SLAB, TAIL, CNTPOP, CNTVISIT, LEAFREQ, "s87", "s84", "s85", "s88", "s86", "s89", "s79", "s76", "s77", "s80", "s78", "s81"); break;            \
-	case 2: SNAIL_DESCEND_PF2(PRE, ORGOPS, SLAB, TAIL, CNTPOP, CNTVISIT, LEAFREQ, "s84", "s87", "s88", "s85", "s86", "s89", "s76", "s79", "s80", "s77", "s78", "s81"); break;            \
-	case 3: SNAIL_DESCEND_PF2(PRE, ORGOPS, SLAB, TAIL, CNTPOP, CNTVISIT, LEAFREQ, "s87", "s84", "s88", "s85", "s86", "s89", "s79", "s76", "s80", "s77", "s78", "s81"); break;            \
-	case 4: SNAIL_DESCEND_PF2(PRE, ORGOPS, SLAB, TAIL, CNTPOP, CNTVISIT, LEAFREQ, "s84", "s87", "s85", "s88", "s89", "s86", "s76", "s79", "s77", "s80", "s81", "s78"); break;            \
-	case 5: SNAIL_DESCEND_PF2(PRE, ORGOPS, SLAB, TAIL, CNTPOP, CNTVISIT, LEAFREQ, "s87", "s84", "s85", "s88", "s89", "s86", "s79", "s76", "s77", "s80", "s81", "s78"); break;            \
-	case 6: SNAIL_DESCEND_PF2(PRE, ORGOPS, SLAB, TAIL, CNTPOP, CNTVISIT, LEAFREQ, "s84", "s87", "s88", "s85", "s89", "s86", "s76", "s79", "s80", "s77", "s81", "s78"); break;            \
-	default: SNAIL_DESCEND_PF2(PRE, ORGOPS, SLAB, TAIL, CNTPOP, CNTVISIT, LEAFREQ, "s87", "s84", "s88", "s85", "s89", "s86", "s79", "s76", "s80", "s77", "s81", "s78"); break;           \
+	case 0: SNAIL_DESCEND_PF2M("0x0e000000", PRE, ORGOPS, SLAB, TAIL, CNTPOP, CNTVISIT, LEAFREQ, "s84", "s87", "s85", "s88", "s86", "s89", "s76", "s79", "s77", "s80", "s78", "s81"); break;            \
+	case 1: SNAIL_DESCEND_PF2M("0x1c000000", PRE, ORGOPS, SLAB, TAIL, CNTPOP, CNTVISIT, LEAFREQ, "s87", "s84", "s85", "s88", "s86", "s89", "s79", "s76", "s77", "s80", "s78", "s81"); break;            \
+	case 2: SNAIL_DESCEND_PF2M("0x2a000000", PRE, ORGOPS, SLAB, TAIL, CNTPOP, CNTVISIT, LEAFREQ, "s84", "s87", "s88", "s85", "s86", "s89", "s76", "s79", "s80", "s77", "s78", "s81"); break;            \
+	case 3: SNAIL_DESCEND_PF2M("0x38000000", PRE, ORGOPS, SLAB, TAIL, CNTPOP, CNTVISIT, LEAFREQ, "s87", "s84", "s88", "s85", "s86", "s89", "s79", "s76", "s80", "s77", "s78", "s81"); break;            \
+	case 4: SNAIL_DESCEND_PF2M("0x46000000", PRE, ORGOPS, SLAB, TAIL, CNTPOP, CNTVISIT, LEAFREQ, "s84", "s87", "s85", "s88", "s89", "s86", "s76", "s79", "s77", "s80", "s81", "s78"); break;            \
+	case 5: SNAIL_DESCEND_PF2M("0x54000000", PRE, ORGOPS, SLAB, TAIL, CNTPOP, CNTVISIT, LEAFREQ, "s87", "s84", "s85", "s88", "s89", "s86", "s79", "s76", "s77", "s80", "s81", "s78"); break;            \
+	case 6: SNAIL_DESCEND_PF2M("0x62000000", PRE, ORGOPS, SLAB, TAIL, CNTPOP, CNTVISIT, LEAFREQ, "s84", "s87", "s88", "s85", "s89", "s86", "s76", "s79", "s80", "s77", "s81", "s78"); break;            \
+	default: SNAIL_DESCEND_PF2M("0x70000000", PRE, ORGOPS, SLAB, TAIL, CNTPOP, CNTVISIT, LEAFREQ, "s87", "s84", "s88", "s85", "s89", "s86", "s79", "s76", "s80", "s77", "s81", "s78"); break;           \
 	}
 
 #define SNAIL_DESCEND_OCT(PRE, ORGOPS, SLAB, TAIL, CNTPOP, CNTVISIT, OCT)                                                                     \
@@ -1145,7 +1173,7 @@
 			if(COH) {
 				if(SHADOW && REL) { SNAIL_DESCEND_PF2_OCT(SNAIL_PRE_NONE_X, SNAIL_ORG_SHARED, SNAIL_SLAB_COH_R, SNAIL_TAIL_ANY, "", SNAIL_COUNT, SNAIL_PF_LEAFREQ_SLOT0, oct) }
 				else if(SHADOW) { SNAIL_DESCEND_PF2_OCT(SNAIL_PRE_SHARED, SNAIL_ORG_SHARED, SNAIL_SLAB_COH, SNAIL_TAIL_ANY, "", SNAIL_COUNT, SNAIL_PF_LEAFREQ_TRI, oct) }
-				else if(POSDIST) { SNAIL_DESCEND_PF2_OCT(SNAIL_PRE_NONE_X, SNAIL_ORG_SHARED, SNAIL_SLAB_COH_R, SNAIL_TAIL_POS, SNAIL_COUNT, "", SNAIL_PF_LEAFREQ_SLOT0, oct) }
+				else if(POSDIST) { SNAIL_DESCEND_PF2_OCT(SNAIL_PRE_NONE_X, SNAIL_ORG_SHARED, SNAIL_SLAB_COH_R, SNAIL_TAIL_POSF, SNAIL_COUNT, "", SNAIL_PF_LEAFREQ_SLOT0, oct) }
 				else { SNAIL_DESCEND_PF2_OCT(SNAIL_PRE_SHARED, SNAIL_ORG_SHARED, SNAIL_SLAB_COH, SNAIL_TAIL_ANY, SNAIL_COUNT, "", SNAIL_PF_LEAFREQ_TRI, oct) }
 			} else {
 				if(SHADOW && REL) { SNAIL_DESCEND_PF2_PLAIN(SNAIL_PRE_NONE_X, SNAIL_ORG_SHARED, SNAIL_SLAB_FAST_R, SNAIL_TAIL_ANY, "", SNAIL_COUNT, SNAIL_PF_LEAFREQ_SLOT0); }
@@ -2625,7 +2653,14 @@
 	return in;
 }
 __host__ __device__ inline unsigned relAux(const unsigned (&rel)[6], unsigned sub, unsigned aux) {
-	return !(sub & 0x80000000u) && (aux & 7u) && relOriginInside(rel) ? aux | (1u << SNAIL_REL_INSIDE_BIT) : aux;
+	const bool leaf = (sub & 0x80000000u) != 0;
+	if(!leaf && !(aux & 7u)) return aux;
+	unsigned bits = 0;
+	for(int c = 0; c < 3; c++) {
+		if(__builtin_bit_cast(float, rel[c]) > 0.0f) bits |= 1u << (SNAIL_REL_NEARPOS_BIT + c);
+		if(__builtin_bit_cast(float, rel[3 + c]) < 0.0f) bits |= 1u << (SNAIL_REL_FARNEG_BIT + c);
+	}
+	return !leaf && relOriginInside(rel) ? aux | (1u << SNAIL_REL_INSIDE_BIT) : aux | bits;
 }
 __global__ __launch_bounds__(256) void k_rel_nodes(const uint4 *__restrict__ pf, int nSlots, float ox, float oy, float oz, uint4 *__restrict__ rel) {
 	const int i = (int)(blockIdx.x * 256 + threadIdx.x);
@@ -2662,6 +2697,14 @@
 	const bool flagged = i < nSlots && !(rel[(size_t)i * 2 + 1].z & 0x80000000u) && ((rel[(size_t)i * 2 + 1].w >> SNAIL_REL_INSIDE_BIT) & 1u);
 	const u64 m = __builtin_amdgcn_ballot_w64(flagged);
 	if((threadIdx.x & 63) == 0 && m) atomicAdd(out, (unsigned long long)__builtin_popcountll(m));
+}
+__global__ __launch_bounds__(256) void k_rel_axis_flag_count(const uint4 *__restrict__ rel, int nSlots, unsigned long long *__restrict__ out) {
+	const int i = (int)(blockIdx.x * 256 + threadIdx.x);
+	const unsigned w = i < nSlots ? rel[(size_t)i * 2 + 1].w : 0u;
+	for(int k = 0; k < 3; k++) {
+		const u64 lo = __builtin_amdgcn_ballot_w64((w >> (SNAIL_REL_NEARPOS_BIT + 2 * k)) & 1u), hi = __builtin_amdgcn_ballot_w64((w >> (SNAIL_REL_NEARPOS_BIT + 2 * k + 1)) & 1u);
+		if((threadIdx.x & 63) == 0 && (lo | hi)) atomicAdd(out + k, (unsigned long long)__builtin_popcountll(lo) | (unsigned long long)__builtin_popcountll(hi) << 32);
+	}
 }
 #endif
 
diff --git a/snail_amd/csrc/snail_hip.hip b/snail_amd/csrc/snail_hip.hip
--- a/snail_amd/csrc/snail_hip.hip
+++ b/snail_amd/csrc/snail_hip.hip
@@ -681,6 +681,10 @@
 }
 
 static size_t pfTrisOffset(int) { return (size_t)1 << 25; }
+static bool pfFits(size_t nSlots, size_t nTris) {
+	const size_t pfBytes = pfTrisOffset(0) + nTris * 64;
+	return nSlots < ((size_t)1 << 20) && pfBytes < ((size_t)1 << 31) && nTris <= (size_t)SNAIL_REL_COUNT_MASK;
+}
 
 SnailScene *snail_scene_create(const void *nodes32, int nNodes, const void *tris64, int nTris, int depth, int device) {
 	if(!nodes32 || !tris64 || nNodes <= 0 || nTris <= 0) { snail_set_error("snail_scene_create: empty scene"); return nullptr; }
@@ -741,7 +745,7 @@
 	SnailScene *s = new SnailScene();
 	s->device = device; s->nNodes = nNodes; s->nTris = nTris; s->depth = realDepth; s->fastOK = fastOK; s->nestedOK = nestedOK;
 	const size_t trisOff = pfTrisOffset(nNodes), pfBytes = trisOff + (size_t)nTris * 64;
-	const bool fits = (size_t)nNodes + 1 < ((size_t)1 << 20) && pfBytes < ((size_t)1 << 31);
+	const bool fits = pfFits((size_t)nNodes + 1, (size_t)nTris);
 	s->pfOKButNesting = pairsOdd && fits;
 	s->pfOK = s->pfOKButNesting && nestedOK;
 	s->trisOff = (int)(fits ? trisOff : 0);
@@ -784,7 +788,7 @@
 	s->device = device; s->nNodes = 2 * nTris - 1; s->nTris = nTris; s->depth = depth; s->fastOK = fastOK;
 	s->dNodes = dNodes;
 	const size_t trisOff = pfTrisOffset(s->nNodes), pfBytes = trisOff + (size_t)nTris * 64;
-	const bool fits = (size_t)s->nNodes + 1 < ((size_t)1 << 20) && pfBytes < ((size_t)1 << 31);
+	const bool fits = pfFits((size_t)s->nNodes + 1, (size_t)nTris);
 	s->trisOff = (int)(fits ? trisOff : 0);
 	s->nestedOK = 1; s->pfOKButNesting = s->pfOK = fits ? 1 : 0;
 	hipError_t e;
@@ -1573,6 +1577,32 @@
 	return 0;
 }
 
+int snail_debug_rel_axis_flag_count(SnailScene *s, const float org[3], int out[6]) {
+	if(int rc = checkScene(s, "snail_debug_rel_axis_flag_count")) return rc;
+	if(!org || !out) { snail_set_error("snail_debug_rel_axis_flag_count: null argument"); return 1; }
+	if(!stackPack(s)) { snail_set_error("snail_debug_rel_axis_flag_count: this scene keeps no origin-relative node records"); return 1; }
+	DeviceGuard guard(s->device);
+	HostCallScope hc(s, "snail_debug_rel_axis_flag_count");
+	if(hc.rc) return hc.rc;
+	if(int rc = hc.zeroStats()) return rc;
+	{
+		SNAIL_LOCK(s);
+		SceneUse use(s, hc.stream());
+		if(use.rc) return use.rc;
+		const uint4 *rel = nullptr;
+		int which = -1;
+		if(int rc = relFor(s, org, hc.stream(), &rel, &which)) return rc;
+		const int nSlots = s->nNodes + 1;
+		hipLaunchKernelGGL(dev::k_rel_axis_flag_count, dim3((unsigned)((nSlots + 255) / 256)), dim3(256), 0, hc.stream(), rel, nSlots, (unsigned long long *)hc.stats());
+		HIP_TRY(hipGetLastError());
+		if(int rc = relUsed(s, which, hc.stream())) return rc;
+	}
+	uint64_t st[4] = {0, 0, 0, 0};
+	if(int rc = hc.finish(st)) return rc;
+	for(int k = 0; k < 3; k++) { out[2 * k] = (int)(st[k] & 0xffffffffu); out[2 * k + 1] = (int)(st[k] >> 32); }
+	return 0;
+}
+
 #endif
 
 int snail_account_packets(SnailScene *s, const float cam[13], int resx, int resy, uint32_t *out8) {
```
